# bpatchasaheb/mayaMatchMoveSolver

Hardware: AMD Instinct MI355X
Metric: LM iterations/sec + residuals/sec (markers x frames) at 1/2/4/8 MI355X; final RMS reproj error (higher is better)
Workload: dtype f64; 1 GPU; c4_500pose_50kbnd_200kobs; frames=500, cameras=1, bundles=50000, markers=50000, observations=200000, parameters=152991, residuals=400000, parallelism=single, solver=lmder fwd-FD delta=1e-4 tau=1 tol=1e-6

## Files before the change

include/mmba.h:

```cpp
#ifndef MMBA_H
#define MMBA_H

#include <stddef.h>
#include <stdint.h>

#ifdef __cplusplus
extern "C" {
#endif

#define MMBA_ABI_VERSION 12

#define MMBA_OK 0
#define MMBA_ERR_INVALID (-1)
#define MMBA_ERR_DEVICE (-2)
#define MMBA_ERR_UNSUPPORTED (-3)
#define MMBA_ERR_INTERRUPTED (-4)
#define MMBA_ERR_NO_DEVICE (-5)
#define MMBA_ERR_COMM (-6)

#define MMBA_SOLVER_CMINPACK_LMDIF 1
#define MMBA_SOLVER_CMINPACK_LMDER 2

#define MMBA_SCENE_GRAPH_MAYA_DAG 1
#define MMBA_SCENE_GRAPH_MM_SCENE_GRAPH 2
// ... 178 lines not shown
                                       double offset, double scale);
double mmba_param_internal_to_external(double value, double xmin, double xmax,
                                       double offset, double scale);

int mmba_context_create(int device, mmba_context **out);
int mmba_context_create_multi(const int *devices, int ndevices, mmba_context **out);
int mmba_context_num_devices(const mmba_context *ctx);
void mmba_context_destroy(mmba_context *ctx);
int mmba_context_synchronize(mmba_context *ctx);
int mmba_host_alloc(size_t bytes, void **out);
void mmba_host_free(void *p);

int mmba_plan_create(mmba_context *ctx, const mmba_problem *prob,
                     const mmba_options *opt, mmba_plan **out);
void mmba_plan_destroy(mmba_plan *plan);

typedef struct mmba_comm mmba_comm;
int mmba_comm_unique_id(unsigned char out_id[128]);
int mmba_comm_create_rccl(mmba_context *ctx, int rank, int nranks,
                          const unsigned char unique_id[128], mmba_comm **out);
int mmba_comm_create_local(int nranks, mmba_comm **out);
void mmba_comm_destroy(mmba_comm *comm);
int mmba_comm_count(const mmba_comm *comm);
int mmba_plan_create_sharded(mmba_context *ctx, const mmba_problem *prob,
                             const mmba_options *opt, mmba_comm *comm, mmba_plan **out);
int mmba_plan_num_shards(const mmba_plan *plan);
int mmba_shard_layout(int32_t num_frames, int32_t num_obs, const int32_t *obs_frame,
                      const int32_t *obs_bundle, int32_t num_bundles, int32_t nranks,
                      int32_t *bounds_out , int32_t *bundle_owner_out);

int mmba_plan_set_attr_values(mmba_plan *plan, const double *attr_values);

int mmba_plan_measure(mmba_plan *plan, const double *x, double *fvec_out,
                      double *err_user_out, double *err_dist_out,
                      double *avg_min_max_out );

int mmba_plan_reproject(mmba_plan *plan, const double *x, double *point_xy_out,
                        double *marker_xy_out);

int mmba_plan_jacobian(mmba_plan *plan, const double *x, double *fjac);

int mmba_plan_solve(mmba_plan *plan, double *x_inout, double *fvec_out,
                    double *err_user_out, double *err_dist_out,
                    mmba_result *res, const mmba_callbacks *cb,
                    mmba_trace *trace);

int mmba_plan_outputs(mmba_plan *plan, double *fvec_out, double *err_user_out,
                      double *err_dist_out);

int mmba_solve_per_frame(mmba_context *ctx, const mmba_problem *prob,
                         const mmba_options *opt, double *x_inout,
                         mmba_result *results , int32_t max_concurrency,
                         const mmba_callbacks *cb);

int mmba_plan_solve_per_frame(mmba_plan *plan, double *x_inout, mmba_result *results,
                              const mmba_callbacks *cb);

int mmba_solve(mmba_context *ctx, const mmba_problem *prob,
               const mmba_options *opt, double *x_inout, double *fvec_out,
               double *err_user_out, double *err_dist_out, mmba_result *res,
               const mmba_callbacks *cb, mmba_trace *trace);

typedef struct mmba_kernel_stats {
    double jac_ms_avg;
    double jac_bytes;
    int32_t jac_launches;
    double resid_ms_avg;
    double resid_bytes;
    int32_t resid_launches;
    double chol_ms_avg;
    double chol_flops;
    int32_t chol_launches;
    int32_t reduced_dim;
    int32_t reduced_kind;
    int32_t dataflow_fallback;
    int32_t shards_replicated;
    int32_t spec_replays;
    int32_t band_solver;
    int32_t band_levels;
    int32_t band_block;
    double chol_flops_alg;
    int32_t pre_handbacks;
    int32_t ne_split_launches;
} mmba_kernel_stats;
int mmba_plan_kernel_stats(mmba_plan *plan, int enable_timing,
                           mmba_kernel_stats *out);

#define MMBA_PATH_PCR 1
#define MMBA_PATH_SHARD_BCR 2
#define MMBA_PATH_BCR_DATAFLOW 3
#define MMBA_PATH_BCR_GRID 4
#define MMBA_PATH_DENSE 5
#define MMBA_PATH_PERFRAME_BATCH 6
#define MMBA_PATH_LOCAL_RING 7
#define MMBA_PATH_PROBE 8
#define MMBA_PATH_SHARD_SEP 9
#define MMBA_PATH_TRIAL_RECORDS 10
#define MMBA_PATH_LENS_CF 11
#define MMBA_PATH_DEST_LANE 12
#define MMBA_PATH_FAULT_SHARD 13
#define MMBA_PATH_COMM_TIMEOUT_MS 14
#define MMBA_PATH_STALL_SHARD 15
#define MMBA_PATH_PCR_CHAIN 16
#define MMBA_PATH_BACKSUB_ONEPASS 17
#define MMBA_PATH_JB_RECOMPUTE 18
#define MMBA_PATH_NE_CF_SPLIT 19
#define MMBA_PATH_RED_BD 20
#define MMBA_PATH_HANDBACK_DMA 21
#define MMBA_PATH_PRE_HANDBACK 22
#define MMBA_PATH_PRE_SCHUR 23
#define MMBA_PATH_BACKSUB_GROUP 24
#define MMBA_PATH_NUM 25
int mmba_debug_set_path(int key, int value);

int mmba_debug_band_solve(mmba_context *ctx, int nb, int w, int nG, int P, const double *S,
                          const double *r, double *x, double *ynorm2, int *parts_used);
int mmba_debug_comm_allreduce(mmba_context *ctx, mmba_comm *comm, double *buf, int count,
                              int op);
int mmba_debug_dgemm(mmba_context *ctx, int tri, int in_place, int M, int N, int K,
                     const double *A, int lda, const double *B, int ldb, double *C, int ldc,
                     double alpha, double beta);

int mmba_debug_reduced_residual(mmba_plan *plan, const double *x, double lam, double *relres);

int mmba_debug_damped_step(mmba_plan *plan, const double *x, double lam, double *step_out,
                           double *g_out, double *diag_out, double *fjac_out);

#ifdef __cplusplus
}
#endif

#endif
```

mayamatchmovesolver_amd/abi.py:

```python
import ctypes as C

MMBA_OK = 0
MMBA_ERR_INVALID = -1
MMBA_ERR_DEVICE = -2
MMBA_ERR_UNSUPPORTED = -3
MMBA_ERR_INTERRUPTED = -4
MMBA_ERR_NO_DEVICE = -5
MMBA_ERR_COMM = -6

SOLVER_TYPE_CMINPACK_LMDIF = 1
SOLVER_TYPE_CMINPACK_LMDER = 2
SCENE_GRAPH_MODE_MAYA_DAG = 1
SCENE_GRAPH_MODE_MM_SCENE_GRAPH = 2
AUTO_DIFF_TYPE_FORWARD = 0
AUTO_DIFF_TYPE_CENTRAL = 1
ROBUST_LOSS_TYPE_TRIVIAL = 0
ROBUST_LOSS_TYPE_SOFT_L_ONE = 1
ROBUST_LOSS_TYPE_CAUCHY = 2
ABI_VERSION = 12

PATH_PCR = 1
PATH_SHARD_BCR = 2
PATH_BCR_DATAFLOW = 3
PATH_BCR_GRID = 4
PATH_DENSE = 5
PATH_PERFRAME_BATCH = 6
PATH_LOCAL_RING = 7
PATH_PROBE = 8
PATH_SHARD_SEP = 9
PATH_TRIAL_RECORDS = 10
PATH_LENS_CF = 11
PATH_DEST_LANE = 12
PATH_FAULT_SHARD = 13
PATH_COMM_TIMEOUT_MS = 14
PATH_STALL_SHARD = 15
PATH_PCR_CHAIN = 16
PATH_BACKSUB_ONEPASS = 17
PATH_JB_RECOMPUTE = 18
PATH_NE_CF_SPLIT = 19
PATH_RED_BD = 20
PATH_HANDBACK_DMA = 21
PATH_PRE_HANDBACK = 22
PATH_PRE_SCHUR = 23
PATH_BACKSUB_GROUP = 24
PATH_NUM = 25

FILM_FIT_FILL = 0
FILM_FIT_HORIZONTAL = 1
FILM_FIT_VERTICAL = 2
FILM_FIT_OVERSCAN = 3

ROO_XYZ, ROO_YZX, ROO_ZXY, ROO_XZY, ROO_YXZ, ROO_ZYX = range(6)

LENS_NONE = 0
LENS_3DE_CLASSIC = 1
LENS_3DE_RADIAL_STD_DEG4 = 2
LENS_3DE_ANAMORPHIC_STD_DEG4 = 3
LENS_3DE_ANAMORPHIC_STD_DEG4_RESCALED = 4

CAM_FILM_BACK_W_INCH = 0
CAM_FILM_BACK_H_INCH = 1
CAM_FOCAL_MM = 2
CAM_FILM_OFFSET_X_INCH = 3
CAM_FILM_OFFSET_Y_INCH = 4
CAM_NEAR_CLIP = 5
CAM_FAR_CLIP = 6
CAM_SCALE = 7
CAM_NUM_ATTRS = 8
LENS_NUM_ATTRS = 14

_i32p = C.POINTER(C.c_int32)
_i64p = C.POINTER(C.c_int64)
_f64p = C.POINTER(C.c_double)


class MmbaProblem(C.Structure):
    _fields_ = [
        ("num_frames", C.c_int32),
        ("num_attrs", C.c_int32),
        ("attr_animated", _i32p),
        ("attr_offset", _i64p),
        ("attr_values", _f64p),
        ("num_transforms", C.c_int32),
        ("tfm_parent", _i32p),
        ("tfm_rotate_order", _i32p),
        ("tfm_attrs", _i32p),
        ("num_cameras", C.c_int32),
        ("cam_tfm", _i32p),
        ("cam_attrs", _i32p),
        ("cam_film_fit", _i32p),
        ("cam_render_size", _i32p),
        ("cam_lens", _i32p),
        ("num_lenses", C.c_int32),
        ("lens_type", _i32p),
        ("lens_attrs", _i32p),
        ("num_bundles", C.c_int32),
        ("bnd_tfm", _i32p),
        ("num_markers", C.c_int32),
        ("mkr_cam", _i32p),
        ("mkr_bnd", _i32p),
        ("num_obs", C.c_int32),
        ("obs_marker", _i32p),
        ("obs_frame", _i32p),
        ("obs_xy", _f64p),
        ("obs_weight", _f64p),
        ("num_params", C.c_int32),
        ("param_attr", _i32p),
        ("param_frame", _i32p),
        ("param_min", _f64p),
        ("param_max", _f64p),
        ("param_offset", _f64p),
        ("param_scale", _f64p),
        ("param_weight", _f64p),
        ("num_stiff", C.c_int32),
        ("stiff_attr", _i32p),
        ("stiff_frame", _i32p),
        ("stiff_weight", _f64p),
        ("stiff_variance", _f64p),
        ("stiff_value", _f64p),
        ("num_smooth", C.c_int32),
        ("smooth_attr", _i32p),
        ("smooth_frame", _i32p),
        ("smooth_weight", _f64p),
        ("smooth_variance", _f64p),
        ("smooth_value", _f64p),
        ("cam_rs_value", _f64p),
        ("lens_input", _i32p),
        ("lens_input_values", _f64p),
# ... 18 lines not shown
        ("scene_graph_mode", C.c_int32),
        ("image_width", C.c_double),
        ("accept_only_better", C.c_int32),
        ("log_level", C.c_int32),
        ("robust_loss", C.c_int32),
        ("robust_loss_type", C.c_int32),
        ("robust_loss_scale", C.c_double),
        ("initial_error_given", C.c_int32),
        ("pad_opt0", C.c_int32),
        ("initial_error_avg", C.c_double),
    ]


class MmbaResult(C.Structure):
    _fields_ = [
        ("success", C.c_int32),
        ("reason_number", C.c_int32),
        ("iterations", C.c_int32),
        ("function_evals", C.c_int32),
        ("jacobian_evals", C.c_int32),
        ("outer_iterations", C.c_int32),
        ("user_interrupted", C.c_int32),
        ("error_is_better", C.c_int32),
        ("error_final", C.c_double),
        ("error_avg", C.c_double),
        ("error_min", C.c_double),
        ("error_max", C.c_double),
        ("error_initial_avg", C.c_double),
        ("error_rms", C.c_double),
        ("num_trace", C.c_int32),
        ("pad0", C.c_int32),
        ("time_solve_s", C.c_double),
        ("time_func_s", C.c_double),
        ("time_jac_s", C.c_double),
        ("time_linear_s", C.c_double),
    ]

    def as_dict(self):
        return {name: getattr(self, name) for name, _ in self._fields_ if name != "pad0"}


INTERRUPT_FN = C.CFUNCTYPE(C.c_int, C.c_void_p)
PROGRESS_FN = C.CFUNCTYPE(None, C.c_void_p, C.c_int)


class MmbaCallbacks(C.Structure):
    _fields_ = [
        ("interrupt", INTERRUPT_FN),
        ("progress", PROGRESS_FN),
        ("user", C.c_void_p),
    ]


class MmbaTrace(C.Structure):
    _fields_ = [
        ("fnorm", _f64p),
        ("capacity", C.c_int32),
        ("count", C.c_int32),
    ]


class MmbaKernelStats(C.Structure):
    _fields_ = [
        ("jac_ms_avg", C.c_double),
        ("jac_bytes", C.c_double),
        ("jac_launches", C.c_int32),
        ("resid_ms_avg", C.c_double),
        ("resid_bytes", C.c_double),
        ("resid_launches", C.c_int32),
        ("chol_ms_avg", C.c_double),
        ("chol_flops", C.c_double),
        ("chol_launches", C.c_int32),
        ("reduced_dim", C.c_int32),
        ("reduced_kind", C.c_int32),
        ("dataflow_fallback", C.c_int32),
        ("shards_replicated", C.c_int32),
        ("spec_replays", C.c_int32),
        ("band_solver", C.c_int32),
        ("band_levels", C.c_int32),
        ("band_block", C.c_int32),
        ("chol_flops_alg", C.c_double),
        ("pre_handbacks", C.c_int32),
        ("ne_split_launches", C.c_int32),
    ]

    def as_dict(self):
        return {name: getattr(self, name) for name, _ in self._fields_}


EXPORTED_SYMBOLS = [
    "mmba_abi_version",
    "mmba_device_count",
    "mmba_last_error",
    "mmba_options_default",
    "mmba_param_external_to_internal",
    "mmba_param_internal_to_external",
    "mmba_context_create",
    "mmba_context_create_multi",
    "mmba_context_num_devices",
    "mmba_plan_num_shards",
    "mmba_debug_damped_step",
    "mmba_debug_reduced_residual",
    "mmba_context_destroy",
    "mmba_context_synchronize",
    "mmba_host_alloc",
    "mmba_host_free",
    "mmba_plan_create",
    "mmba_plan_destroy",
    "mmba_comm_unique_id",
    "mmba_shard_layout",
    "mmba_comm_create_rccl",
    "mmba_comm_create_local",
    "mmba_comm_destroy",
    "mmba_comm_count",
    "mmba_plan_create_sharded",
    "mmba_plan_measure",
    "mmba_plan_reproject",
    "mmba_solve_per_frame",
    "mmba_plan_solve_per_frame",
    "mmba_plan_set_attr_values",
    "mmba_plan_jacobian",
    "mmba_plan_solve",
    "mmba_plan_outputs",
    "mmba_solve",
    "mmba_plan_kernel_stats",
    "mmba_debug_set_path",
    "mmba_debug_band_solve",
    "mmba_debug_comm_allreduce",
    "mmba_debug_dgemm",
]
```

mayamatchmovesolver_amd/csrc/mmba_api.cpp:

```cpp
#include <atomic>
#include <cfloat>
#include <cmath>
#include <cstring>
#include <string>

#include "mmba_geom.h"
#include "mmba_kernels.h"
#include "mmba_plan.h"

namespace mmba {
static thread_local std::string g_last_error;
void set_error(const std::string &msg) { g_last_error = msg; }

static_assert(MMBA_PATH_NUM == 25, "one initialiser per path key");
static std::atomic<int> g_path[MMBA_PATH_NUM] = {-1, -1, -1, -1, -1, -1, -1, -1, -1, -1, -1, -1, -1,
                                                 -1, -1, -1, -1, -1, -1, -1, -1, -1, -1, -1, -1};
int path_choice(int key) {
    return (key > 0 && key < MMBA_PATH_NUM) ? g_path[key].load() : -1;
}
}

using namespace mmba;

#define MMBA_GUARD(...)                               \
    try {                                             \
        __VA_ARGS__                                   \
    } catch (const DeviceError &) {                   \
        return MMBA_ERR_DEVICE;                       \
    } catch (const CommError &) {                     \
        return MMBA_ERR_COMM;                         \
    } catch (const Unsupported &u) {                  \
        set_error("unsupported: " + u.what);          \
        return MMBA_ERR_UNSUPPORTED;                  \
    } catch (const Invalid &v) {                      \
        set_error("invalid: " + v.what);              \
        return MMBA_ERR_INVALID;                      \
    } catch (const std::exception &e) {               \
        set_error(std::string("exception: ") + e.what()); \
        return MMBA_ERR_INVALID;                      \
    }

extern "C" {

int mmba_abi_version(void) { return MMBA_ABI_VERSION; }

int mmba_debug_set_path(int key, int value) {
    if (key <= 0 || key >= MMBA_PATH_NUM) return MMBA_ERR_INVALID;
    g_path[key].store(value < 0 ? -1 : value);
    return MMBA_OK;
}

int mmba_shard_layout(int32_t num_frames, int32_t num_obs, const int32_t *obs_frame,
                      const int32_t *obs_bundle, int32_t num_bundles, int32_t nranks,
                      int32_t *bounds_out, int32_t *bundle_owner_out) {
    if (num_frames <= 0 || num_obs < 0 || nranks <= 0 || !bounds_out ||
        (num_obs > 0 && !obs_frame) || (bundle_owner_out && (!obs_bundle || num_bundles < 0)))
        return MMBA_ERR_INVALID;
    for (int i = 0; i < num_obs; ++i) {
        if (obs_frame[i] < 0 || obs_frame[i] >= num_frames) return MMBA_ERR_INVALID;
        if (bundle_owner_out && (obs_bundle[i] < 0 || obs_bundle[i] >= num_bundles))
            return MMBA_ERR_INVALID;
    }
    mmba::shard_layout(num_frames, num_obs, obs_frame, obs_bundle, num_bundles, nranks,
                       bounds_out, bundle_owner_out);
    return MMBA_OK;
}

const char *mmba_last_error(void) { return g_last_error.c_str(); }

int mmba_device_count(void) {
    int count = 0;
    if (hipGetDeviceCount(&count) != hipSuccess) return 0;
    int ok = 0;
    for (int d = 0; d < count; ++d) {
        hipDeviceProp_t prop;
        if (hipGetDeviceProperties(&prop, d) != hipSuccess) continue;
        if (std::strncmp(prop.gcnArchName, "gfx950", 6) == 0) ++ok;
    }
    return ok;
}

void mmba_options_default(mmba_options *o, int32_t solver_type) {
    if (!o) return;
    std::memset(o, 0, sizeof(*o));
    o->solver_type = solver_type ? solver_type : MMBA_SOLVER_CMINPACK_LMDER;
    o->iter_max = 100;
    o->tau = 1.0;
    o->eps1 = 1e-6;
    o->eps2 = 1e-6;
    o->eps3 = 1e-6;
    o->delta = 1e-4;
    o->auto_diff_type = MMBA_AUTO_DIFF_FORWARD;
    o->auto_param_scale = 1;
    o->scene_graph_mode = MMBA_SCENE_GRAPH_MAYA_DAG;
    o->image_width = 2048.0;
    o->accept_only_better = 1;
    o->log_level = 0;
}

// ... 223 lines not shown
                    mmba_trace *trace) {
    if (!plan || !x_inout) return MMBA_ERR_INVALID;
    if (plan->group)
        return group_plan_solve(plan, x_inout, fvec_out, err_user_out, err_dist_out, res, cb,
                                trace);
    MMBA_GUARD({
        MMBA_HIP(hipSetDevice(plan->impl.ctx->device));
        plan->impl.outputs_ready = false;
        const int rc =
            plan->impl.solve(x_inout, fvec_out, err_user_out, err_dist_out, res, cb, trace);
        plan->impl.outputs_ready = rc == MMBA_OK || rc == MMBA_ERR_INTERRUPTED;
        return rc;
    })
}

int mmba_plan_outputs(mmba_plan *plan, double *fvec_out, double *err_user_out,
                      double *err_dist_out) {
    if (plan && plan->group) return group_plan_outputs(plan, fvec_out, err_user_out, err_dist_out);
    if (!plan || !plan->impl.outputs_ready) return MMBA_ERR_INVALID;
    MMBA_GUARD({
        Plan &p = plan->impl;
        MMBA_HIP(hipSetDevice(p.ctx->device));
        if (fvec_out || err_user_out || err_dist_out)
            p.download_ref_order(p.d_f, p.d_eu, p.d_ed, fvec_out, err_user_out, err_dist_out);
        return MMBA_OK;
    })
}

int mmba_plan_set_attr_values(mmba_plan *plan, const double *attr_values) {
    if (!plan || !attr_values) return MMBA_ERR_INVALID;
    if (plan->group) return group_plan_set_attr_values(plan, attr_values);
    MMBA_GUARD({
        Plan &p = plan->impl;
        MMBA_HIP(hipSetDevice(p.ctx->device));
        std::memcpy(p.host_attr0.data(), attr_values, p.attr_bytes);
        MMBA_HIP(hipMemcpyAsync(p.d_attr0, p.host_attr0.data(), p.attr_bytes,
                                hipMemcpyHostToDevice, p.s));
        MMBA_HIP(hipStreamSynchronize(p.s));
        return MMBA_OK;
    })
}

int mmba_plan_solve_per_frame(mmba_plan *plan, double *x_inout, mmba_result *results,
                              const mmba_callbacks *cb) {
    if (!plan || !x_inout || !results) return MMBA_ERR_INVALID;
    if (plan->group) return group_plan_solve_per_frame(plan, x_inout, results, cb);
    MMBA_GUARD({
        MMBA_HIP(hipSetDevice(plan->impl.ctx->device));
        plan->impl.outputs_ready = false;
        return plan->impl.solve_frames(x_inout, results, cb);
    })
}

int mmba_solve(mmba_context *ctx, const mmba_problem *prob, const mmba_options *opt,
               double *x_inout, double *fvec_out, double *err_user_out, double *err_dist_out,
               mmba_result *res, const mmba_callbacks *cb, mmba_trace *trace) {
    mmba_plan *plan = nullptr;
    int rc = mmba_plan_create(ctx, prob, opt, &plan);
    if (rc != MMBA_OK) return rc;
    rc = mmba_plan_solve(plan, x_inout, fvec_out, err_user_out, err_dist_out, res, cb, trace);
    mmba_plan_destroy(plan);
    return rc;
}

int mmba_plan_kernel_stats(mmba_plan *plan, int enable_timing, mmba_kernel_stats *out) {
    if (!plan) return MMBA_ERR_INVALID;
    if (plan->group) return group_plan_kernel_stats(plan, enable_timing, out);
    Plan &p = plan->impl;
    if (out) {
        std::memset(out, 0, sizeof(*out));
        out->jac_launches = p.jac_n;
        out->jac_ms_avg = p.jac_n ? p.jac_ms / p.jac_n : 0.;
        out->resid_launches = p.resid_n;
        out->resid_ms_avg = p.resid_n ? p.resid_ms / p.resid_n : 0.;
        out->chol_launches = p.chol_n;
        out->chol_ms_avg = p.chol_n ? p.chol_ms / p.chol_n : 0.;
        out->reduced_dim = p.nR;
        out->reduced_kind = p.band ? (p.bs.use_bd ? 3 : 0) : (p.dense ? 2 : 1);
        out->dataflow_fallback = p.bs.df_off ? 1 : 0;
        out->shards_replicated = p.replicated ? 1 : 0;
        out->spec_replays = p.spec_replays;
        out->pre_handbacks = (int32_t)p.pre_handbacks;
        out->ne_split_launches = (int32_t)p.ne_split_launches;
        {
            const BandSolver &b = p.bs;
            out->band_solver = !p.band ? 0
                               : b.use_bd ? 5
                               : (b.pcr_int && !b.df_off) ? 4
                               : (b.use_pcr && !b.df_off) ? 3
                               : b.use_bcr ? 2
                               : 1;
        }
        double bj = 0.;
        {
            const double pc = p.ncf ? (double)p.nCF / p.ncf : 0.;
            const double pb = p.nB ? 3.0 * p.nB_solved / p.nB : 0.;
            const double pg = (double)std::min(p.nG, NGMAX);
            bj = 48.0 + 8.0 * pc * (pb + pg);
        }
        out->jac_bytes = bj * p.M;
        out->resid_bytes = 48.0 * p.M;
        if (p.band && p.bs.use_pcr && !p.bs.df_off) {
            const double K = p.bs.pcr.K;
            out->chol_flops = (double)p.bs.pcr.nblk *
                              (p.bs.pcr.nlev * (28.0 / 3.0 * K * K * K + 9.0 * K * K) + 2.0 * K * K);
        } else if (p.band && p.bs.use_bcr) {
            const double K = p.bs.bcr.K, G = p.bs.bcr.nG, N = p.bs.bcr.NR;
            out->chol_flops = (p.bs.bcr.nblk - 1) * (19.0 / 3.0 * K * K * K + 5.0 * G * K * K +
                                                     G * G * K + K * K) +
                              2.0 * N * N * N / 3.0;
        } else if (p.band && p.bs.use_bd) {
            const double pc = p.ncf ? (double)p.nCF / p.ncf : 0.;
            out->chol_flops = (double)p.nCF * pc * pc / 3.0;
        } else if (p.band) {
            out->chol_flops = (double)(p.nR - p.nG) * p.bw * p.bw;
        } else {
            out->chol_flops = (double)p.nRpad * p.nRpad * p.nRpad / 3.0;
        }
        {
            const double G = p.nG, nb = p.nR - p.nG;
            const double arrow = nb * G * (2.0 * p.bw + G) + G * G * G / 3.0 + 4.0 * G * G;
            if (p.band && p.bs.use_bd) {
                const double pc = p.ncf ? (double)p.nCF / p.ncf : 0.;
                out->chol_flops_alg = (double)p.ncf * (pc * pc * pc / 3.0 + 4.0 * pc * pc) +
                                      nb * G * (2.0 * pc + G) + G * G * G / 3.0 + 4.0 * G * G;
            } else if (p.band) {
                out->chol_flops_alg = nb * p.bw * p.bw + 4.0 * nb * p.bw + arrow;
            } else {
                const double N = p.nR;
                out->chol_flops_alg = N * N * N / 3.0 + 4.0 * N * N;
            }
            if (p.band && p.bs.use_pcr && !p.bs.df_off) {
                out->band_levels = p.bs.pcr.nlev;
                out->band_block = p.bs.pcr.K;
            } else if (p.band && p.bs.use_bcr) {
                out->band_levels = 0;
                for (int a = p.bs.bcr.nblk; a > 1; a = (a + 1) / 2) ++out->band_levels;
                out->band_block = p.bs.bcr.K;
            }
        }
    }
    p.timing = enable_timing != 0;
    if (enable_timing) {
        p.jac_ms = p.resid_ms = p.chol_ms = 0.;
        p.jac_n = p.resid_n = p.chol_n = 0;
        p.span_ctr[0] = p.span_ctr[1] = p.span_ctr[2] = 0;
    }
    return MMBA_OK;
}

int mmba_debug_reduced_residual(mmba_plan *plan, const double *x, double lam, double *relres) {
    if (!plan || !x || !relres || lam < 0.) return MMBA_ERR_INVALID;
    if (plan->group) {
        set_error("unsupported: reduced residual hook on a multi-device plan");
        return MMBA_ERR_UNSUPPORTED;
    }
    MMBA_GUARD({
        Plan &p = plan->impl;
        MMBA_HIP(hipSetDevice(p.ctx->device));
        p.outputs_ready = false;
        return p.reduced_residual(x, lam, relres);
    })
}

int mmba_debug_damped_step(mmba_plan *plan, const double *x, double lam, double *step_out,
                           double *g_out, double *diag_out, double *fjac_out) {
// ... 123 lines not shown
```

mayamatchmovesolver_amd/csrc/mmba_kernels.h:

```cpp
#pragma once

#include <vector>

#include "mmba_internal.h"

namespace mmba {

constexpr int NE_BND_TPB = 64;

void launch_param_prep(hipStream_t s, const DevProblem &P, const double *x, double *ext,
                       double *ext_pert, double *step, int solver_type, double delta,
                       double eps_dif);
void launch_set_attrs(hipStream_t s, const DevProblem &P, const double *ext);
void launch_param_set(hipStream_t s, const DevProblem &P, const double *x, double *ext,
                      double *ext_pert, double *step, int solver_type, double delta,
                      double eps_dif);
struct RedRow {
    int off, n, is_max, slot;
};
struct RedSpec {
    int nrows;
    int flag_slot;
    RedRow row[8];
};
// ... 23 lines not shown
int trial_blocks(const DevProblem &P);
void launch_reproject(hipStream_t s, const DevProblem &P, const double *recs, double *pts,
                      double *mkr);
void launch_residual(hipStream_t s, const DevProblem &P, const double *recs, double *f, double *eu,
                     double *ed, double *partial, double *out = nullptr,
                     unsigned int *ticket = nullptr, double *dist = nullptr);
void launch_dist_stats(hipStream_t s, const DevProblem &P, const double *ed, double *partial,
                       int nparts, int rstride, double *out);
struct RedTail {
    int on = 0;
    RedSpec spec{};
    const double *partial = nullptr;
    double *scalar = nullptr;
    int *flag = nullptr;
    double *host = nullptr;
    int host_n = 0;
    unsigned *ticket = nullptr;
};
void launch_residual_jp(hipStream_t s, const DevProblem &P, const double *recs, double *f,
                        double *eu, double *ed, double *partial, const double *J,
                        const int *jcol, const int *nloc, const double *pstep,
                        double *partial_jp, double *dist = nullptr, const RedTail &T = RedTail());
struct CentralB {
    const double *recs = nullptr, *brec = nullptr, *ext_pert = nullptr, *step = nullptr;
    const double *q15 = nullptr, *kap15 = nullptr;
};
void launch_param_central(hipStream_t s, const DevProblem &P, const double *x, double *ext_pertB,
                          double *stepB, double delta, double *count, double *c15 = nullptr);
void launch_b15_s(hipStream_t s, const double *fsq, double fn, double *out);
void launch_b15_combine(hipStream_t s, int n, const double *u, const double *c, const double *zu,
                        const double *zc, const double *sp, double *xs, double *kinv,
                        double *scalar, int fail_slot, const double *fail_prev);
void launch_b15_q(hipStream_t s, const DevProblem &P, const double *c, double *q15, double *kap15,
                  double *cr);
void launch_b15_rot(hipStream_t s, const DevProblem &P, const double *q15, const double *x,
                    double *out);
void launch_b15_accl(hipStream_t s, const DevProblem &P, const double *Acc, const double *q15,
                     const double *diag, double lam, double *AccL, double *diagL);
void launch_b15_unrot(hipStream_t s, const DevProblem &P, const double *Acc, const double *g,
                      const double *q15, double *adiag, double *u);
void launch_b15_unrot_J(hipStream_t s, const DevProblem &P, double *J, const double *q15);
void launch_b15_dnorm(hipStream_t s, int n, const double *x, const double *diag, double *out);
void launch_b15_newton(hipStream_t s, int n, const double *v, const double *zu, const double *zc,
                       const double *kinv, double *out);
void launch_b15_jp(hipStream_t s, int n, const double *xs, const double *u, const double *c,
                   const double *sp, double *out);
void launch_jacobian(hipStream_t s, const DevProblem &P, const double *recs,
                     const double *ext_pert, const double *step, int solver_type, double *J,
                     int *jcol, int *nloc, const int *stale_param, double *eu, double *ed,
                     int ncv = 0,
                     const double *f = nullptr,
                     const CentralB &CB = CentralB());
void launch_rows_eval(hipStream_t s, const DevProblem &P, double *fr, double *eur,
                      double *partial, int slot, const double *Jrow = nullptr,
                      const double *pstep = nullptr, double *partial_jp = nullptr);
void launch_rows_jac(hipStream_t s, const DevProblem &P, const double *ext,
                     const double *ext_pert, const double *step, const double *ext_pertB,
                     const double *stepB, int lmder, double *Jrow, double *eur, int last_param);
void launch_rows_ne(hipStream_t s, const DevProblem &P, const double *Jrow, const double *fr,
                    const int *p_own, double *Acc, double *Abb, double *aggbuf, double *g);
constexpr int NE_CF_SPLIT = 4;
constexpr int NE_CF_NT = 36;
struct NeEpi {
    int on = 0;
    int first = 0, mode = 1, do_xn = 0, do_gn = 0;
    double fnorm = 0.;
    const double *fnorm_sq = nullptr;
    const double *x = nullptr;
    double *diag = nullptr, *acnorm = nullptr, *partial = nullptr;
    int rstride = 0, cf_base = 0, bnd_base = 0;
    int fold = 0;
    RedSpec spec{};
    double *scalar = nullptr;
    unsigned *ticket = nullptr;
    const double *jb_recs = nullptr;
    int jb_lmder = 1;
    double *cf_part = nullptr;
    unsigned *cf_ticket = nullptr;
    double *Lb = nullptr, *tb = nullptr;
    int *fail = nullptr;
    const int *gate = nullptr;
    long long *probe = nullptr;
};
bool jac_ne_fusable(const DevProblem &P, int ncv);
void launch_jac_ne(hipStream_t s, const DevProblem &P, const double *recs, const double *step,
                   int solver_type, double *J, int *jcol, int *nloc, const int *stale_param,
                   double *eu, double *ed, double *Acc, double *g, const NeEpi &E);
bool ne_epilogue_fusable(const DevProblem &P);
bool launch_ne(hipStream_t s, const DevProblem &P, const double *J, const int *jcol,
               const int *nloc, const double *f, double *Acc, double *Acg, double *Abb,
               double *Abg, double *aggbuf, double *g, double *glob_partial, int glob_chunk,
               const NeEpi &epi = NeEpi(), bool cf_done = false);
void launch_colnorms(hipStream_t s, const DevProblem &P, const double *Acc, const double *Abb,
                     const double *aggbuf, double *acnorm, double *g);
void launch_bundle_factor(hipStream_t s, const DevProblem &P, const double *Abb,
                          const double *Abg, const double *g, const double *diag, double lam,
                          double *Lb, double *tb, double *Wg, int *fail);
void launch_schur_obs(hipStream_t s, const DevProblem &P, const double *J, const double *Lb,
                      double *W, const RedSpec *red = nullptr, const double *partial = nullptr,
                      double *scalar = nullptr, const int *gate = nullptr);
void launch_schur_obs_rs(hipStream_t s, const DevProblem &PV, int Mr, const int *nloc,
                         const int *vobs, const int *vcoff, const double *J, const double *Lb,
                         double *W);
void launch_schur_init(hipStream_t s, const DevProblem &P, const double *Acc, const double *Acg,
                       const double *Agg, const double *g, const double *diag, double lam,
                       const SView &V, int npad, double *rhs, const RedSpec *red = nullptr,
                       const double *partial = nullptr, double *scalar = nullptr);
void launch_schur_pairs(hipStream_t s, const DevProblem &P, const double *W, const double *Wg,
                        const double *tb, const SView &V, double *rhs);
void launch_chol_panel(hipStream_t s, double *S, const int *slot, int NT, int k, const int *rows,
                       int nrows, double *Linv, int *fail);
void launch_chol_update(hipStream_t s, double *S, const int *slot, int NT, int k,
                        const int2 *pairs, int npairs);
void launch_trsv_fwd(hipStream_t s, const double *S, const int *slot, int NT, int k,
                     const int *rows, int nrows, const double *Linv, double *r, double *y);
void launch_trsv_bwd(hipStream_t s, const double *S, const int *slot, int NT, int k,
                     const int *cols, int ncols, const double *Linv, double *y, double *x);
void launch_trsv_fwd_all(hipStream_t s, const double *S, const int *slot, int NT,
                         const int *rows_off, const int *rows, const double *Linv, double *r,
                         double *y);
void launch_trsv_bwd_all(hipStream_t s, const double *S, const int *slot, int NT,
                         const int *cols_off, const int *cols, const double *Linv, double *y,
                         double *x);
struct SchurInitFold {
    int on;
    const double *Acc, *g, *diag;
    double lam;
};
bool launch_schur_dest(hipStream_t s, const DevProblem &P, const double *W, const int2 *dest,
                       const int *dest_off, int ndest, const int2 *pairs, const SView &V,
                       int pc_uniform, int assign_off, const double *tb = nullptr,
                       double *rhs = nullptr, SchurInitFold fold = SchurInitFold{},
                       const int *wave_list = nullptr, int n_wave = 0,
                       const int *lane_list = nullptr, int n_lane = 0);
void launch_schur_rhs(hipStream_t s, const DevProblem &P, const double *W, const double *tb,
                      const int *row_cf, double *rhs);
void launch_schur_glob(hipStream_t s, const DevProblem &P, const double *W, const double *Wg,
                       const double *tb, const SView &V, double *rhs);
void launch_backsub_bundle(hipStream_t s, const DevProblem &P, const double *W, const double *Wg,
                           const double *tb, const double *Lb, const double *xR, double *U,
                           double *x);
struct TrialFold {
    const double *x = nullptr, *diag = nullptr;
    double *wa1 = nullptr, *wa2 = nullptr, *wa3 = nullptr;
    double *ext = nullptr, *ext_pert = nullptr, *step = nullptr;
    int solver_type = 0;
    double delta = 0., eps_dif = 0.;
    const int *other = nullptr;
    int nother = 0;
    double *partial = nullptr;
    int rstride = 0;
    const int *own = nullptr;
    int rec = 0;
    double *recs = nullptr, *brec = nullptr;
    int group = 0;
    const int2 *bobs_rp = nullptr;
    int brec_fwd = 0;
};
bool trial_records_ok(const DevProblem &P);
int trial_fold_parts(const DevProblem &P, int nother, bool rec = false);
int trial_prep_rec_parts(const DevProblem &P, int nother);
void launch_trial_prep_rec(hipStream_t s, const DevProblem &P, const double *xs, const TrialFold &T);
void launch_obs_wtx(hipStream_t s, const DevProblem &P, const double *W, const double *xR,
                    double *U);
void launch_backsub_trial(hipStream_t s, const DevProblem &P, const double *W, const double *Wg,
                          const double *tb, const double *Lb, const double *xR, const double *U,
                          double *x, const TrialFold &T);
void launch_scatter_xR(hipStream_t s, const DevProblem &P, const double *xR, double *x);
void launch_newton_bundle(hipStream_t s, const DevProblem &P, const double *W, const double *Wg,
                          const double *Lb, const double *v, double *wR, double *usq,
                          double *un, double *gp);
void launch_gather_R(hipStream_t s, const DevProblem &P, const double *v, double *vR, int nRpad);
void band_factor(hipStream_t s, const BandSolver &B, int *fail, long long *probe);
void band_factor_forward(hipStream_t s, const BandSolver &B, int *fail, long long *probe,
                         const double *r, double *y);
void band_forward(hipStream_t s, const BandSolver &B, const double *r, double *y);
void band_backward(hipStream_t s, const BandSolver &B, const double *y, double *x);
void bcr_factor(hipStream_t s, const BandSolver &B, int *fail, long long *probe,
                const double *r = nullptr, double *y = nullptr);
void bcr_forward(hipStream_t s, const BandSolver &B, const double *r, double *y);
void bcr_backward(hipStream_t s, const BandSolver &B, const double *y, double *x);
void pcr_solve(hipStream_t s, const PcrDev &P, const double *r, double *x, double *xs, int *fail);
void pcr_rhs_dot(hipStream_t s, const PcrDev &P, const double *w, const int *mask, int *fail);
void pcr_rhs_mc(hipStream_t s, const PcrDev &P, const double *R, int ldr, int nc, double *Z,
                int ldz, int *fail);
void pcr_note_context(int dev, int delta);
int pcr_max_resident(int K);
int pcr_resident_wide(int K);
int pcr_grid(int nblk);
void bd_direct(hipStream_t s, const DevProblem &P, const BdDev &D, const double *Acc,
               const double *g, const double *diag, double lam, double *xR, double *xs,
               int *fail, double *scalar, int dn_slot, int fail_slot,
               const RedSpec *red = nullptr, const double *partial = nullptr);
void bd_factor_solve(hipStream_t s, const BdDev &D, int *fail, const double *r, double *y,
                     double *x, double *xs);
void bd_forward(hipStream_t s, const BdDev &D, const double *w, double *y);
void launch_sumsq(hipStream_t s, const double *a, const double *d, int n, double *partial,
                  int nparts, double *out, const int *mask = nullptr,
                  unsigned int *ticket = nullptr);
void launch_sumsq_div(hipStream_t s, const double *a, const double *d, int n, double *partial,
                      int nparts, double *out, const int *mask = nullptr,
                      unsigned int *ticket = nullptr);
void launch_sumsq_mix(hipStream_t s, const double *y, const double *v, int n, double *partial,
                      int nparts, double *out, const int *mask);
void launch_reduce_sum(hipStream_t s, const double *partial, int n, double *out);
void launch_gnorm(hipStream_t s, const double *g, const double *acnorm, int n, double fnorm,
                  double *partial, int nparts, double *out, const int *mask = nullptr,
                  unsigned int *ticket = nullptr);
void launch_jp_sumsq(hipStream_t s, const DevProblem &P, const double *J, const int *jcol,
                     const int *nloc, const double *p, double *partial, int nparts,
                     double *out, unsigned int *ticket = nullptr);
void launch_zero_flag(hipStream_t s, const double *acnorm, int n, const int *mask,
                      double *partial, int nparts, double *out, unsigned int *ticket = nullptr);
void launch_flag_to_scalar(hipStream_t s, int *flag, double *out);
void launch_keep_rows(hipStream_t s, double *v, int lo, int hi, int nCF, int nR, int root);
void launch_keep_mask(hipStream_t s, const double *src, const int *mask, int n, double *dst);
void launch_lm_step(hipStream_t s, int n, const double *xs, const double *x, const double *diag,
                    double *wa1, double *wa2, double *wa3);
void launch_diag_init(hipStream_t s, int n, const double *acnorm, double *diag, int first,
                      int mode);
void launch_newton_v(hipStream_t s, int n, const double *diag, const double *x, double dxnorm,
                     double *v);
void launch_handback_host(hipStream_t s, int Mg, int nrows, const int *dev_of_ref,
                          const double *f2, const double *eu2, const double *ed, double *hf,
                          double *heu, double *hed, const double *dec = nullptr,
                          const double *f2_trial = nullptr);
void launch_unpermute(hipStream_t s, int M, const int *ref_of_dev, const int *obs_own,
                      const double *f2,
                      const double *eu2, const double *ed, double *f2o, double *eu2o,
                      double *edo);

void launch_fold_ranks(hipStream_t s, const double *t, int nranks, double *out, int do_xn,
                       int do_gn);

void launch_batch_lm(hipStream_t s, const DevProblem &P, const BatchArgs &B, int nf_max);

void launch_dgemm_nt(hipStream_t s, bool tri, int M, int N, int Kd, const double *A, int lda,
                     const double *B, int ldb, double *C, int ldc, double alpha, double beta);

void launch_jacobian_rs(hipStream_t s, const DevProblem &P, const double *ext_pert,
// ... 8 lines not shown
```

mayamatchmovesolver_amd/csrc/mmba_kernels.hip:

```cpp
#include <cfloat>
#include <cstdlib>

#include "mmba_geom.h"
#include "mmba_kernels.h"
#include "mmba_red_dev.h"

namespace mmba {

MMBA_DEV bool own_obs(const DevProblem &P, int i) { return !P.obs_own || P.obs_own[i]; }
MMBA_DEV bool own_cf(const DevProblem &P, int cf) { return !P.cf_own || P.cf_own[cf]; }
MMBA_DEV bool own_bnd(const DevProblem &P, int b) { return !P.bnd_own || P.bnd_own[b]; }
MMBA_DEV bool own_mask(const int *m, int i) { return !m || m[i]; }

__device__ __forceinline__ int xcd_remap(int b, int G) {
    const int x = b & 7, idx = b >> 3, q = G >> 3, r = G & 7;
    return x * q + min(x, r) + idx;
}

template <bool MAX>
__device__ __forceinline__ void finish_blocks(double v, double *partial, double *out,
                                              unsigned int *ticket, int blk = -1) {
    if (blk < 0) blk = blockIdx.x;
    __shared__ int last;
    __shared__ double red[256];
// ... 10 lines not shown
    if (!ticket) return;
    __syncthreads();
    if (!last) return;
    __threadfence();
    double a = 0.;
    for (int i = threadIdx.x; i < (int)gridDim.x; i += blockDim.x) {
        const double q = __hip_atomic_load(&partial[i], __ATOMIC_RELAXED, __HIP_MEMORY_SCOPE_AGENT);
        a = MAX ? fmax(a, q) : a + q;
    }
    red[threadIdx.x] = a;
    __syncthreads();
    for (int w = 128; w > 0; w >>= 1) {
        if (threadIdx.x < w)
            red[threadIdx.x] = MAX ? fmax(red[threadIdx.x], red[threadIdx.x + w])
                                   : red[threadIdx.x] + red[threadIdx.x + w];
        __syncthreads();
    }
    if (threadIdx.x == 0) {
        *out = red[0];
        __hip_atomic_store(ticket, 0u, __ATOMIC_RELAXED, __HIP_MEMORY_SCOPE_AGENT);
    }
}

__device__ __forceinline__ void bundle_chol3(double (&A)[3][3], double (&rhs)[3],
                                             const double (&dd)[3], int pb, double lam, int b,
                                             double *Lb, double *tb, int *fail,
                                             double (*Lo)[3] = nullptr, double *ilo = nullptr) {
#pragma unroll
    for (int a = 0; a < 3; ++a) {
        if (a < pb) {
            const double d = dd[a];
            A[a][a] += lam * (d * d);
            if (A[a][a] == 0.) {
                A[a][a] = 1.;
                rhs[a] = 0.;
            }
        }
    }
    double L[3][3] = {}, il[3];
    bool ok = true;
#pragma unroll
    for (int j = 0; j < 3; ++j) {
        double s = A[j][j];
#pragma unroll
        for (int k = 0; k < j; ++k) s -= L[j][k] * L[j][k];
        if (!(s > 0.)) {
            ok = false;
            s = 1.;
        }
        L[j][j] = sqrt(s);
        il[j] = 1.0 / L[j][j];
#pragma unroll
        for (int i = j + 1; i < 3; ++i) {
            double t = A[i][j];
#pragma unroll
            for (int k = 0; k < j; ++k) t -= L[i][k] * L[j][k];
            L[i][j] = t * il[j];
        }
    }
    if (!ok) atomicOr(fail, 1);
#pragma unroll
    for (int a = 0; a < 3; ++a)
#pragma unroll
        for (int c = 0; c < 3; ++c) Lb[(size_t)b * 9 + a * 3 + c] = (a < pb) ? L[a][c] : 0.;
    double t[3];
#pragma unroll
    for (int a = 0; a < 3; ++a) {
        double s = rhs[a];
#pragma unroll
        for (int k = 0; k < a; ++k) s -= L[a][k] * t[k];
        t[a] = s * il[a];
    }
    for (int a = 0; a < 3; ++a) tb[(size_t)b * 3 + a] = t[a];
    if (Lo) {
#pragma unroll
        for (int a = 0; a < 3; ++a) {
            ilo[a] = il[a];
#pragma unroll
            for (int c = 0; c < 3; ++c) Lo[a][c] = L[a][c];
        }
    }
}

__device__ __forceinline__ double reduce_row_w64(const double *partial, const RedRow &rw) {
    const bool mx = rw.is_max != 0;
    const int t = threadIdx.x & 63;
    double s[4];
    constexpr int JB = 6;
    if (rw.n <= 256 * JB) {
        double q[4][JB];
#pragma unroll
        for (int k = 0; k < 4; ++k)
#pragma unroll
            for (int j = 0; j < JB; ++j) {
                const int i = t + 64 * k + 256 * j;
                q[k][j] = i < rw.n ? partial[rw.off + i] : 0.;
            }
#pragma unroll
        for (int k = 0; k < 4; ++k) {
            double v = 0.;
#pragma unroll
            for (int j = 0; j < JB; ++j)
                if (t + 64 * k + 256 * j < rw.n) v = mx ? fmax(v, q[k][j]) : v + q[k][j];
            s[k] = v;
        }
    } else {
#pragma unroll
        for (int k = 0; k < 4; ++k) {
            double v = 0.;
            for (int i = t + 64 * k; i < rw.n; i += 256) {
                const double q = partial[rw.off + i];
                v = mx ? fmax(v, q) : v + q;
            }
            s[k] = v;
        }
    }
    const double a0 = mx ? fmax(s[0], s[2]) : s[0] + s[2];
    const double a1 = mx ? fmax(s[1], s[3]) : s[1] + s[3];
    double r = mx ? fmax(a0, a1) : a0 + a1;
#pragma unroll
    for (int w = 32; w > 0; w >>= 1) {
        const double o = __shfl_down(r, w);
        if (t < w) r = mx ? fmax(r, o) : r + o;
    }
    return r;
}

constexpr int RED_ROWS = 8;
__device__ __forceinline__ void reduce_rows_sc1(const RedSpec &spec, const double *partial,
                                                double *scalar) {
    __shared__ double red[RED_ROWS][256];
    const int nr = spec.nrows;
    double sv[RED_ROWS];
#pragma unroll
    for (int r = 0; r < RED_ROWS; ++r) {
        sv[r] = 0.;
        if (r < nr) {
            const RedRow rw = spec.row[r];
            const bool mx = rw.is_max != 0;
            for (int i = threadIdx.x; i < rw.n; i += blockDim.x) {
                const double q = ld_sc1(&partial[rw.off + i]);
                sv[r] = mx ? fmax(sv[r], q) : sv[r] + q;
            }
        }
    }
#pragma unroll
    for (int r = 0; r < RED_ROWS; ++r)
        if (r < nr) red[r][threadIdx.x] = sv[r];
    __syncthreads();
    for (int w = 128; w > 0; w >>= 1) {
        if (threadIdx.x < w) {
#pragma unroll
            for (int r = 0; r < RED_ROWS; ++r) {
                if (r >= nr) break;
                const bool mx = spec.row[r].is_max != 0;
                red[r][threadIdx.x] = mx ? fmax(red[r][threadIdx.x], red[r][threadIdx.x + w])
                                         : red[r][threadIdx.x] + red[r][threadIdx.x + w];
            }
        }
        __syncthreads();
    }
    if (threadIdx.x < nr) scalar[spec.row[threadIdx.x].slot] = red[threadIdx.x][0];
    __syncthreads();
}

__device__ __forceinline__ void tail_reduce(const RedSpec &spec, const double *partial,
                                            double *scalar, unsigned *ticket) {
    __shared__ unsigned last;
    asm volatile("s_waitcnt vmcnt(0)" ::: "memory");
    __syncthreads();
    if (threadIdx.x == 0)
        last = __hip_atomic_fetch_add(ticket, 1u, __ATOMIC_RELAXED, __HIP_MEMORY_SCOPE_AGENT) ==
               gridDim.x - 1;
    __syncthreads();
    if (!last) return;
    reduce_rows_sc1(spec, partial, scalar);
    if (threadIdx.x == 0) __hip_atomic_store(ticket, 0u, __ATOMIC_RELAXED, __HIP_MEMORY_SCOPE_AGENT);
}

__device__ __forceinline__ void tail_reduce_full(const RedTail &T) {
    __shared__ unsigned last;
    asm volatile("s_waitcnt vmcnt(0)" ::: "memory");
    __syncthreads();
    if (threadIdx.x == 0)
        last = __hip_atomic_fetch_add(T.ticket, 1u, __ATOMIC_RELAXED, __HIP_MEMORY_SCOPE_AGENT) ==
               gridDim.x - 1;
    __syncthreads();
    if (!last) return;
    reduce_rows_sc1(T.spec, T.partial, T.scalar);
    if (threadIdx.x == 0 && T.flag && T.spec.flag_slot >= 0) {
        T.scalar[T.spec.flag_slot] = (double)*T.flag;
        *T.flag = 0;
    }
    if (T.host) {
        asm volatile("s_waitcnt vmcnt(0)" ::: "memory");
        __syncthreads();
        for (int i = threadIdx.x; i < T.host_n; i += blockDim.x) T.host[i] = ld_sc1(&T.scalar[i]);
    }
    if (threadIdx.x == 0)
        __hip_atomic_store(T.ticket, 0u, __ATOMIC_RELAXED, __HIP_MEMORY_SCOPE_AGENT);
}

__device__ __forceinline__ void param_prep_one(const DevProblem &P, int p, double v, double *ext,
                                               double *ext_pert, double *step, int solver_type,
                                               double delta, double eps_dif) {
    const double xmin = P.p_min[p], xmax = P.p_max[p], off = P.p_off[p], sc = P.p_scale[p];
    ext[p] = int_to_ext(v, xmin, xmax, off, sc);
    double st;
// ... 700 lines not shown
        __syncthreads();
        for (int t = threadIdx.x; t < 2 * lm * NE_CHUNK; t += blockDim.x) {
            const int row = t / NE_CHUNK, o = t % NE_CHUNK;
            sJ[row][o] = (o < cnt) ? J[(size_t)row * M + c0 + o] : 0.;
        }
        if (nG > 0) {
            for (int t = threadIdx.x; t < NGMAX * NE_CHUNK; t += blockDim.x)
                sG[t / NE_CHUNK][t % NE_CHUNK] = -1;
            __syncthreads();
            for (int t = threadIdx.x; t < lm * NE_CHUNK; t += blockDim.x) {
                const int l = t / NE_CHUNK, o = t % NE_CHUNK;
                if (o >= cnt || l < pc || l >= nloc[c0 + o]) continue;
                const int p = jcol[(size_t)l * M + c0 + o];
                if (P.p_class[p] == PC_G) sG[P.p_pos[p] - nCF][o] = l;
            }
        }
        for (int t = threadIdx.x; t < NE_CHUNK; t += blockDim.x) {
            sF[0][t] = (t < cnt) ? f[2 * (c0 + t)] : 0.;
            sF[1][t] = (t < cnt) ? f[2 * (c0 + t) + 1] : 0.;
        }
        __syncthreads();
        if (kind == 0) {
            for (int o = 0; o < cnt; ++o)
                acc += sJ[2 * ea][o] * sJ[2 * eb][o] + sJ[2 * ea + 1][o] * sJ[2 * eb + 1][o];
        } else if (kind == 1) {
            for (int o = 0; o < cnt; ++o)
                acc += sJ[2 * ea][o] * sF[0][o] + sJ[2 * ea + 1][o] * sF[1][o];
        } else if (kind == 2) {
            for (int o = 0; o < cnt; ++o) {
                const int l = sG[eb][o];
                if (l >= 0)
                    acc += sJ[2 * ea][o] * sJ[2 * l][o] + sJ[2 * ea + 1][o] * sJ[2 * l + 1][o];
            }
        }
    }
    double *A = &Acc[(size_t)cf * PCMAX * PCMAX];
    if (kind == 0) {
        A[ea * PCMAX + eb] = acc;
        A[eb * PCMAX + ea] = acc;
    } else if (kind == 1) {
        g[P.cf_var_param[P.cf_var_off[cf] + 1 + ea]] = acc;
    } else if (kind == 2) {
        Acg[((size_t)cf * PCMAX + ea) * NGMAX + eb] = acc;
    }
}

__device__ __forceinline__ double epi_param(const NeEpi &E, int p, double d, double gp, double &zf,
                                          double &xn, double &gm) {
    const double an = sqrt(d);
    E.acnorm[p] = an;
    double dg = E.diag[p];
    if (E.mode != 2) {
        if (E.first) dg = an == 0. ? 1. : an;
        dg = fmax(dg, an);
        E.diag[p] = dg;
    }
    if (an == 0.) zf = 1.;
    if (E.do_xn) {
        const double v = dg * E.x[p];
        xn += v * v;
    }
    if (E.do_gn && an != 0.) {
        const double fn = E.fnorm_sq ? sqrt(*E.fnorm_sq) : E.fnorm;
        if (fn != 0.) gm = fmax(gm, fabs((gp / fn) / an));
    }
    return dg;
}

__device__ __forceinline__ void epi_store(const NeEpi &E, int col, double zf, double xn,
                                          double gm) {
    E.partial[col] = zf;
    E.partial[E.rstride + col] = xn;
    E.partial[2 * E.rstride + col] = gm;
}

struct EpiPre {
    int p;
    double dg;
    double xv;
    double fn;
};
template <int PC>
__device__ __forceinline__ EpiPre epi_preload(const DevProblem &P, const NeEpi &E, int cf,
                                              int lane) {
    EpiPre q{-1, 0., 0., 0.};
    if (!E.on || lane >= PC) return q;
    q.p = P.cf_var_param[P.cf_var_off[cf] + 1 + lane];
    q.dg = E.diag[q.p];
    if (E.do_xn) q.xv = E.x[q.p];
    if (E.do_gn) q.fn = E.fnorm_sq ? sqrt(*E.fnorm_sq) : E.fnorm;
    return q;
}
__device__ __forceinline__ void epi_param_pre(const NeEpi &E, const EpiPre &q, double d, double gp,
                                              double &zf, double &xn, double &gm) {
    const double an = sqrt(d);
    E.acnorm[q.p] = an;
    double dg = q.dg;
    if (E.mode != 2) {
        if (E.first) dg = an == 0. ? 1. : an;
        dg = fmax(dg, an);
        E.diag[q.p] = dg;
    }
    if (an == 0.) zf = 1.;
    if (E.do_xn) {
        const double v = dg * q.xv;
        xn += v * v;
    }
    if (E.do_gn && an != 0.) {
        if (q.fn != 0.) gm = fmax(gm, fabs((gp / q.fn) / an));
    }
}
template <int PC>
__device__ __forceinline__ void epi_params_wave(const DevProblem &P, const NeEpi &E, int cf,
                                                int lane, double d, double gp, const EpiPre &q) {
    double zf = 0., xn = 0., gm = 0.;
    if (lane < PC) epi_param_pre(E, q, d, gp, zf, xn, gm);
    double Z = 0., X = 0., G = 0.;
#pragma unroll
    for (int a = 0; a < PC; ++a) {
        const double za = __shfl(zf, a), xa = __shfl(xn, a), ga = __shfl(gm, a);
        if (za != 0.) Z = 1.;
        X += xa;
        G = fmax(G, ga);
    }
    if (lane == 0) epi_store(E, E.cf_base + cf, Z, X, G);
}


template <int PC, int NW, int NG>
__device__ __forceinline__ void ne_cf_u_body(const DevProblem &P, const double *__restrict__ J,
                                             const int *__restrict__ jcol,
                                             const int *__restrict__ nloc,
                                             const double *__restrict__ f, double *Acc,
                                             double *Acg, double *g, const NeEpi &E, int blk,
                                             int nblk_cf) {
    constexpr int NCC = PC * (PC + 1) / 2, NE = NCC + PC, NT = NE + PC * NG;
    __shared__ double wsum[NW][NT];
    const int cf = xcd_remap(blk, nblk_cf);
    if (!own_cf(P, cf) || P.cf_pc[cf] != PC) {
        if (E.on && threadIdx.x == 0) epi_store(E, E.cf_base + cf, 0., 0., 0.);
        return;
    }
    const int o0 = P.cf_obs_off[cf], o1 = P.cf_obs_off[cf + 1];
    const size_t M = P.M;
    const int nCF = P.nR - P.nG;
    const int tid = threadIdx.x, lane = tid & 63, wv = tid >> 6;
    const EpiPre epq = epi_preload<PC>(P, E, cf, lane);
    double acc[NT];
#pragma unroll
    for (int e = 0; e < NT; ++e) acc[e] = 0.;
    for (int i = o0 + tid; i < o1; i += 64 * NW) {
        double jx[PC], jy[PC];
#pragma unroll
        for (int a = 0; a < PC; ++a) {
            jx[a] = J[(2 * a) * M + i];
            jy[a] = J[(2 * a + 1) * M + i];
        }
        const double fx = f[2 * i], fy = f[2 * i + 1];
        int e = 0;
#pragma unroll
        for (int a = 0; a < PC; ++a)
#pragma unroll
            for (int c = a; c < PC; ++c) acc[e++] += jx[a] * jx[c] + jy[a] * jy[c];
#pragma unroll
        for (int a = 0; a < PC; ++a) acc[NCC + a] += jx[a] * fx + jy[a] * fy;
        if constexpr (NG > 0) {
            double gx[NG], gy[NG];
#pragma unroll
            for (int q = 0; q < NG; ++q) gx[q] = gy[q] = 0.;
            const int nl = nloc[i];
            for (int l = PC; l < nl; ++l) {
                const int p = jcol[(size_t)l * M + i];
                if (P.p_class[p] != PC_G) continue;
// ... 84 lines not shown
        double jx[PC], jy[PC];
#pragma unroll
        for (int a = 0; a < PC; ++a) {
            jx[a] = J[(2 * a) * M + i];
            jy[a] = J[(2 * a + 1) * M + i];
        }
        const double fx = f[2 * i], fy = f[2 * i + 1];
        int e = 0;
#pragma unroll
        for (int a = 0; a < PC; ++a)
#pragma unroll
            for (int c = a; c < PC; ++c) acc[e++] += jx[a] * jx[c] + jy[a] * jy[c];
#pragma unroll
        for (int a = 0; a < PC; ++a) acc[NCC + a] += jx[a] * fx + jy[a] * fy;
    }
#pragma unroll
    for (int e = 0; e < NT; ++e) {
        double v = acc[e];
#pragma unroll
        for (int off = 32; off > 0; off >>= 1) v += __shfl_xor(v, off);
        if (lane == 0) wsum[wv][e] = v;
    }
    __syncthreads();
    double *mine = E.cf_part + ((size_t)cf * NS + part) * NE_CF_NT;
    for (int e = tid; e < NT; e += 64 * NW) {
        double v = wsum[0][e];
#pragma unroll
        for (int w = 1; w < NW; ++w) v += wsum[w][e];
        st_sc1(&mine[e], v);
    }
    asm volatile("s_waitcnt vmcnt(0)" ::: "memory");
    __syncthreads();
    if (tid == 0)
        last_s = (__hip_atomic_fetch_add(&E.cf_ticket[cf], 1u, __ATOMIC_ACQ_REL,
                                         __HIP_MEMORY_SCOPE_AGENT) %
                  NS) == NS - 1;
    __syncthreads();
    if (!last_s) return;
    __builtin_amdgcn_fence(__ATOMIC_ACQUIRE, "agent");
    const double *all = E.cf_part + (size_t)cf * NS * NE_CF_NT;
    for (int e = tid; e < NT; e += 64 * NW) {
        double t[NS];
#pragma unroll
        for (int q = 0; q < NS; ++q) t[q] = ld_sc1(&all[(size_t)q * NE_CF_NT + e]);
        double v = t[0];
#pragma unroll
        for (int q = 1; q < NS; ++q) v += t[q];
        fin[e] = v;
    }
    __syncthreads();
    double *A = &Acc[(size_t)cf * PCMAX * PCMAX];
    for (int e = tid; e < NT; e += 64 * NW) {
        const double v = fin[e];
        if (e < NCC) {
            int a = 0, rem = e;
            while (rem >= PC - a) {
                rem -= PC - a;
                ++a;
            }
            const int c = a + rem;
            A[a * PCMAX + c] = v;
            A[c * PCMAX + a] = v;
        } else {
            g[P.cf_var_param[P.cf_var_off[cf] + 1 + (e - NCC)]] = v;
        }
    }
    if (E.on && wv == 0) {
        const int ed = lane * PC - lane * (lane - 1) / 2;
        epi_params_wave<PC>(P, E, cf, lane, lane < PC ? fin[ed] : 0., lane < PC ? fin[NCC + lane] : 0.,
                            epq);
    }
}

template <int PC, int NW, int NG>
__global__ void __launch_bounds__(64 * NW) k_ne_cf_u(DevProblem P, const double *__restrict__ J,
                                                     const int *__restrict__ jcol,
                                                     const int *__restrict__ nloc,
                                                     const double *__restrict__ f, double *Acc,
                                                     double *Acg, double *g, NeEpi E) {
    ne_cf_u_body<PC, NW, NG>(P, J, jcol, nloc, f, Acc, Acg, g, E, blockIdx.x, gridDim.x);
}


template <int PC, int NW, bool GEN>
__global__ void __launch_bounds__(64 * NW) k_jac_ne_u(
    DevProblem P, const double *__restrict__ recs, const double *__restrict__ step,
    int solver_type, double *__restrict__ J, int *__restrict__ jcol, int *__restrict__ nloc,
    const int *__restrict__ stale_param, double *__restrict__ eu, double *__restrict__ ed,
    double *Acc, double *g, NeEpi E) {
    constexpr int NCC = PC * (PC + 1) / 2, NE = NCC + PC;
    __shared__ double wsum[NW][NE];
    __shared__ double sRec[(PC + 1) * CAMREC];
    __shared__ int sPv[PC];
    __shared__ double sSt[PC];
    __shared__ int sHdr[3];
    if (E.gate && __hip_atomic_load(E.gate, __ATOMIC_RELAXED, __HIP_MEMORY_SCOPE_AGENT) == 0)
        return;
    const int cf = xcd_remap(blockIdx.x, gridDim.x);
    long long *pr = (E.probe && threadIdx.x == 0) ? E.probe + 5 * (size_t)cf : nullptr;
    if (pr) pr[0] = (long long)wall_clock64();
    const int o0 = P.cf_obs_off[cf], o1 = P.cf_obs_off[cf + 1];
    const int tid = threadIdx.x, lane = tid & 63, wv = tid >> 6;
    const bool lmder = solver_type == MMBA_SOLVER_CMINPACK_LMDER;
    const bool solved = P.cf_pc[cf] == PC && own_cf(P, cf);
    {
        const int voff = P.cf_var_off[cf];
        const int nv = min(P.cf_var_off[cf + 1] - voff - 1, PC);
        for (int t = tid; t < (nv + 1) * CAMREC; t += 64 * NW)
            sRec[t] = recs[(size_t)voff * CAMREC + t];
        if (tid < PC) {
            const int p = tid < nv ? P.cf_var_param[voff + 1 + tid] : -1;
            sPv[tid] = p;
            sSt[tid] = tid < nv ? step[p] : 1.;
        }
        if (tid == 0) {
            const int fr = P.cf_frame[cf];
            sHdr[0] = nv;
            sHdr[1] = fr;
            sHdr[2] = stale_param[fr];
        }
    }
    __syncthreads();
    if (pr) pr[1] = (long long)wall_clock64();
    JacCf<PC> C;
    C.rcf = sRec;
#pragma unroll
    for (int v = 0; v < PC; ++v) {
        C.pv[v] = sPv[v];
        C.st[v] = sSt[v];
    }
    C.nv = sHdr[0];
    C.fr = sHdr[1];
    C.pstale = sHdr[2];
    double acc[NE];
#pragma unroll
    for (int e = 0; e < NE; ++e) acc[e] = 0.;
    for (int i = o0 + tid; i < o1; i += 64 * NW) {
        double jx[PC], jy[PC], fx, fy;
        int z = 0;
        asm volatile("" : "+s"(z));
        C.rcf = sRec + z;
        jac_obs_u<PC, GEN>(P, i, C, lmder, J, jcol, nloc, eu, ed, jx, jy, fx, fy);
        int e = 0;
#pragma unroll
        for (int a = 0; a < PC; ++a)
#pragma unroll
            for (int c = a; c < PC; ++c) acc[e++] += jx[a] * jx[c] + jy[a] * jy[c];
#pragma unroll
        for (int a = 0; a < PC; ++a) acc[NCC + a] += jx[a] * fx + jy[a] * fy;
    }
    if (pr) pr[2] = (long long)wall_clock64();
    if (!solved) {
        if (E.on && tid == 0) epi_store(E, E.cf_base + cf, 0., 0., 0.);
        if (pr) pr[3] = pr[2];
        return;
    }
#pragma unroll
    for (int e = 0; e < NE; ++e) {
        double v = acc[e];
#pragma unroll
        for (int off = 32; off > 0; off >>= 1) v += __shfl_xor(v, off);
        if (lane == 0) wsum[wv][e] = v;
    }
    __syncthreads();
    double *A = &Acc[(size_t)cf * PCMAX * PCMAX];
    for (int e = tid; e < NE; e += 64 * NW) {
        double v = wsum[0][e];
#pragma unroll
        for (int w = 1; w < NW; ++w) v += wsum[w][e];
        if (e < NCC) {
            int a = 0, rem = e;
            while (rem >= PC - a) {
                rem -= PC - a;
                ++a;
            }
            const int c = a + rem;
            A[a * PCMAX + c] = v;
            A[c * PCMAX + a] = v;
        } else {
            g[P.cf_var_param[P.cf_var_off[cf] + 1 + (e - NCC)]] = v;
        }
    }
    if (E.on && (tid >> 6) == 0) {
        const int ln = tid & 63;
        double d = 0., gp = 0.;
        if (ln < PC) {
            const int ed2 = ln * PC - ln * (ln - 1) / 2;
            d = wsum[0][ed2];
            gp = wsum[0][NCC + ln];
#pragma unroll
            for (int w = 1; w < NW; ++w) {
                d += wsum[w][ed2];
                gp += wsum[w][NCC + ln];
            }
        }
        epi_params_wave<PC>(P, E, cf, ln, d, gp, epi_preload<PC>(P, E, cf, ln));
    }
    if (pr) {
        pr[3] = (long long)wall_clock64();
        unsigned xcc;
        asm volatile("s_getreg_b32 %0, hwreg(HW_REG_XCC_ID)" : "=s"(xcc));
        pr[4] = (long long)(xcc & 0xf);
    }
}

__global__ void __launch_bounds__(NE_BND_TPB) k_ne_bnd_jb(DevProblem P, double *Abb, double *g,
                                                          NeEpi E) {
    __shared__ double red[3][NE_BND_TPB];
    if (E.gate && __hip_atomic_load(E.gate, __ATOMIC_RELAXED, __HIP_MEMORY_SCOPE_AGENT) == 0)
        return;
    const int b = xcd_remap(blockIdx.x, gridDim.x) * blockDim.x + threadIdx.x;
    const int4 p4 = b < P.nB ? P.bnd_p4[b] : make_int4(-1, -1, -1, 0);
    const int pb = p4.w;
    double zf = 0., xn = 0., gm = 0.;
    if (pb > 0) {
        double A[PBMAX][PBMAX] = {};
        double gb[PBMAX] = {};
        const int q0 = P.bobs_off[b], q1 = P.bobs_off[b + 1];
        const double *__restrict__ br = &P.brec[(size_t)b * BREC];
        for (int qb = q0; qb < q1; qb += 4) {
            double4 u[4], v[4];
            if (E.jb_recs) {
                const double bp0[3] = {br[0], br[1], br[2]};
#pragma unroll
                for (int r = 0; r < 4; ++r) {
                    if (qb + r >= q1) break;
                    const int i = P.bobs[qb + r];
                    const double *__restrict__ rec0 = &E.jb_recs[(size_t)P.cf_var_off[P.obs_cf[i]] * CAMREC];
                    const double mx = P.obs_xy[2 * i], my = P.obs_xy[2 * i + 1], sw = P.obs_sqrtw[i];
                    const double2 f0 = residual_e(rec0, bp0, mx, my, sw, P.mode, P.image_width);
                    double jb[6] = {0., 0., 0., 0., 0., 0.};
#pragma unroll
                    for (int a = 0; a < 3; ++a) {
                        if (a < pb) {
                            const double bq[3] = {br[3 + 3 * a], br[4 + 3 * a], br[5 + 3 * a]};
                            const double2 rr = residual_e(rec0, bq, mx, my, sw, P.mode, P.image_width);
                            const double st = br[12 + a];
                            jb[2 * a] = E.jb_lmder ? (rr.x - f0.x) * st : (rr.x - f0.x) / st;
                            jb[2 * a + 1] = E.jb_lmder ? (rr.y - f0.y) * st : (rr.y - f0.y) / st;
                        }
                    }
                    u[r] = make_double4(jb[0], jb[1], jb[2], jb[3]);
                    v[r] = make_double4(jb[4], jb[5], f0.x, f0.y);
                }
            } else {
#pragma unroll
                for (int r = 0; r < 4; ++r) {
                    if (qb + r < q1) {
                        const double4 *src = reinterpret_cast<const double4 *>(&P.JB[(size_t)(qb + r) * 8]);
                        u[r] = src[0];
                        v[r] = src[1];
                    }
                }
            }
#pragma unroll
            for (int r = 0; r < 4; ++r) {
                if (qb + r >= q1) break;
                const double jx[3] = {u[r].x, u[r].z, v[r].x}, jy[3] = {u[r].y, u[r].w, v[r].y};
                const double fx = v[r].z, fy = v[r].w;
#pragma unroll
                for (int a = 0; a < 3; ++a) {
#pragma unroll
                    for (int c = 0; c < 3; ++c) A[a][c] += jx[a] * jx[c] + jy[a] * jy[c];
                    gb[a] += jx[a] * fx + jy[a] * fy;
                }
            }
        }
        double *Ab = &Abb[(size_t)b * 9];
#pragma unroll
        for (int a = 0; a < PBMAX; ++a)
#pragma unroll
            for (int c = 0; c < PBMAX; ++c) Ab[a * 3 + c] = (a < pb && c < pb) ? A[a][c] : 0.;
        g[p4.x] = gb[0];
        if (pb > 1) g[p4.y] = gb[1];
        if (pb > 2) g[p4.z] = gb[2];
        double dd[3] = {0., 0., 0.};
        if (E.on) {
            double zo = 0., xo = 0., go = 0.;
            dd[0] = epi_param(E, p4.x, A[0][0], gb[0], zo, xo, go);
// ... 321 lines not shown
    for (int p = blockIdx.x * blockDim.x + threadIdx.x; p < P.n; p += gridDim.x * blockDim.x) {
        const int cls = P.p_class[p];
        double d = 0.;
        double gp;
        if (cls == PC_CF) {
            const int cf = P.p_blk[p];
            const int a = P.p_pos[p] - P.cf_roff[cf];
            d = Acc[(size_t)cf * PCMAX * PCMAX + a * PCMAX + a];
            gp = g[p];
        } else if (cls == PC_B) {
            const int b = P.p_blk[p];
            const int a = P.p_pos[p];
            d = Abb[(size_t)b * 9 + a * 3 + a];
            gp = g[p];
        } else {
            const int gi = P.p_pos[p] - (P.nR - P.nG);
            d = Agg[gi * NGMAX + gi];
            gp = gG[gi];
            g[p] = gp;
        }
        if (c15) {
            if (cls == PC_CF) {
                d = adiag15[p];
                gp = u15[p];
            }
            const double cp = c15[p];
            d = fmax(d + 2. * cp * gp + s15v * cp * cp, 0.);
            gp = gp + s15v * cp;
            gfull[p] = gp;
        }
        const double an = sqrt(d);
        acnorm[p] = an;
        double dg = diag[p];
        if (mode != 2) {
            if (first) dg = an == 0. ? 1. : an;
            dg = fmax(dg, an);
            diag[p] = dg;
        }
        if (own_mask(mask, p)) {
            if (an == 0.) zf = 1.;
            if (do_xn) {
                const double v = dg * x[p];
                xn += v * v;
            }
            if (do_gn && an != 0.) gm = fmax(gm, fabs((gp / fnorm) / an));
        }
    }
    block_partial<true>(zf, red, partial);
    __syncthreads();
    block_partial<false>(xn, red, partial + rstride);
    __syncthreads();
    block_partial<true>(gm, red, partial + 2 * rstride);
}

__global__ void __launch_bounds__(256) k_trial_prep(
    DevProblem P, const double *__restrict__ xs, const double *__restrict__ x,
    const double *__restrict__ diag, double *wa1, double *wa2, double *wa3, double *ext,
    double *ext_pert, double *step, int solver_type, double delta, double eps_dif,
    const int *__restrict__ mask, double *partial, int rstride) {
    __shared__ double red[256];
    double pn = 0., xn = 0.;
    for (int j = blockIdx.x * blockDim.x + threadIdx.x; j < P.n; j += gridDim.x * blockDim.x) {
        const double st = -xs[j];
        const double dj = diag[j];
        const double xj = x[j] + st;
        const double w3 = dj * st;
        wa1[j] = st;
        wa2[j] = xj;
        wa3[j] = w3;
        param_prep_one(P, j, xj, ext, ext_pert, step, solver_type, delta, eps_dif);
        set_attr_one(P, j, ext[j]);
        if (own_mask(mask, j)) {
            pn += w3 * w3;
            const double v = dj * xj;
            xn += v * v;
        }
    }
    block_partial<false>(pn, red, partial);
    __syncthreads();
    block_partial<false>(xn, red, partial + rstride);
}

__device__ void lm_decide(const LmDec &d, double *scalar) {
    const double p1 = .1, p5 = .5, p25 = .25, p75 = .75, p0001 = 1e-4;
    const double epsmch = DBL_EPSILON;
    double fnorm = d.f0 ? sqrt(scalar[d.s_f0]) : d.fnorm;
    double delta = d.delta, xnorm = d.xnorm, par = d.par, gnorm = d.gnorm;
    int info = 0, go = 0;
    double ratio = 0.;
    bool taken = true;
    if (d.spec) {
        if (d.first) {
            xnorm = sqrt(scalar[d.s_xn2]);
            delta = d.factor * xnorm;
            if (delta == 0.) delta = d.factor;
        }
        gnorm = fnorm != 0. ? scalar[d.s_gnorm] : 0.;
        if (gnorm <= d.gtol) {
            info = 4;
            taken = false;
        } else {
            const double fl = scalar[d.s_fail];
            const bool ok0 = fl == 0.;
            const double dxnorm = ok0 ? sqrt(scalar[d.s_dnorm]) : HUGE_VAL;
            const double fp = dxnorm - delta;
            taken = fl < 2. && fp <= p1 * delta;
            par = 0.;
        }
    }
    if (taken) {
        const double pnorm = sqrt(scalar[d.s_pnorm]);
        if (d.first) delta = fmin(delta, pnorm);
        const double fnorm1 = sqrt(scalar[d.s_fnorm]);
        double actred = -1.;
        if (p1 * fnorm1 < fnorm) {
            const double d1 = fnorm1 / fnorm;
            actred = 1. - d1 * d1;
        }
        const double temp1 = sqrt(scalar[d.s_jp]) / fnorm;
        const double temp2 = (sqrt(par) * pnorm) / fnorm;
        const double prered = temp1 * temp1 + temp2 * temp2 / p5;
        const double dirder = -(temp1 * temp1 + temp2 * temp2);
        if (prered != 0.) ratio = actred / prered;
        if (ratio <= p25) {
            double temp;
            if (actred >= 0.)
                temp = p5;
            else
                temp = p5 * dirder / (dirder + p5 * actred);
            if (p1 * fnorm1 >= fnorm || temp < p1) temp = p1;
            delta = temp * fmin(delta, pnorm / p1);
            par /= temp;
        } else if (par == 0. || ratio >= p75) {
            delta = pnorm / p5;
            par = p5 * par;
        }
        const bool accept = ratio >= p0001;
        if (accept) xnorm = sqrt(scalar[d.s_xn2t]);
        if (fabs(actred) <= d.ftol && prered <= d.ftol && p5 * ratio <= 1.) info = 1;
        if (delta <= d.xtol * xnorm) info = 2;
        if (fabs(actred) <= d.ftol && prered <= d.ftol && p5 * ratio <= 1. && info == 2) info = 3;
        if (info == 0) {
            if (d.nfev >= d.maxfev) info = 5;
            if (fabs(actred) <= epsmch && prered <= epsmch && p5 * ratio <= 1.) info = 6;
            if (delta <= epsmch * xnorm) info = 7;
            if (gnorm <= epsmch) info = 8;
        }
        go = (accept && info == 0) ? 1 : 0;
    }
    scalar[d.s_out] = go;
    scalar[d.s_out + 1] = ratio;
    scalar[d.s_out + 2] = delta;
    scalar[d.s_out + 3] = par;
    scalar[d.s_out + 4] = taken ? info : -100 - info;
    __hip_atomic_store(d.gate, go, __ATOMIC_RELAXED, __HIP_MEMORY_SCOPE_AGENT);
}

__global__ void __launch_bounds__(256) k_reduce_multi(const double *__restrict__ partial,
                                                      RedSpec spec, double *scalar, int *flag,
                                                      double *host, int host_n,
                                                      unsigned *ticket, unsigned *host_seq,
                                                      unsigned seq, const LmDec dec) {
    __shared__ double red[256];
    const RedRow rw = spec.row[blockIdx.x];
    const double v = reduce_row_block<false>(partial, rw, red);
    if (threadIdx.x == 0) {
        scalar[rw.slot] = v;
        if (blockIdx.x == 0 && flag && spec.flag_slot >= 0) {
            scalar[spec.flag_slot] = (double)*flag;
            *flag = 0;
        }
    }
    if (!host && !dec.on) return;
    __shared__ unsigned last;
    if (threadIdx.x == 0) {
        const unsigned t = __hip_atomic_fetch_add(ticket, 1u, __ATOMIC_ACQ_REL,
                                                  __HIP_MEMORY_SCOPE_AGENT);
        last = t == gridDim.x - 1;
    }
    __syncthreads();
    if (!last) return;
    __builtin_amdgcn_fence(__ATOMIC_ACQUIRE, "agent");
    if (dec.on) {
        if (threadIdx.x == 0) lm_decide(dec, scalar);
        __syncthreads();
        __builtin_amdgcn_fence(__ATOMIC_SEQ_CST, "workgroup");
    }
    if (!host) {
        if (threadIdx.x == 0)
            __hip_atomic_store(ticket, 0u, __ATOMIC_RELAXED, __HIP_MEMORY_SCOPE_AGENT);
        return;
    }
    if (threadIdx.x < 64) {
        for (int i = threadIdx.x; i < host_n; i += 64)
            host[i] = __hip_atomic_load(&scalar[i], __ATOMIC_RELAXED, __HIP_MEMORY_SCOPE_AGENT);
        if (host_seq) {
            __threadfence_system();
            if (threadIdx.x == 0)
                __hip_atomic_store(host_seq, seq, __ATOMIC_RELEASE, __HIP_MEMORY_SCOPE_SYSTEM);
        }
    }
    if (threadIdx.x == 0) __hip_atomic_store(ticket, 0u, __ATOMIC_RELAXED, __HIP_MEMORY_SCOPE_AGENT);
}

__global__ void k_bundle_factor(DevProblem P, const double *__restrict__ Abb,
                                const double *__restrict__ Abg, const double *__restrict__ g,
                                const double *__restrict__ diag, double lam, double *Lb,
                                double *tb, double *Wg, int *fail) {
    const int b = xcd_remap(blockIdx.x, gridDim.x) * blockDim.x + threadIdx.x;
    if (b >= P.nB) return;
    const int pb = P.bnd_pb[b];
    if (pb == 0) return;
    const int po = P.bnd_par_off[b];
    double A[3][3], rhs[3], dd[3];
#pragma unroll
    for (int a = 0; a < 3; ++a) {
#pragma unroll
        for (int c = 0; c < 3; ++c)
            A[a][c] = (a < pb && c < pb) ? Abb[(size_t)b * 9 + a * 3 + c] : (a == c ? 1. : 0.);
        rhs[a] = 0.;
        dd[a] = 0.;
        if (a < pb) {
            const int p = P.bnd_par[po + a];
            dd[a] = diag[p];
            rhs[a] = g[p];
        }
    }
    double L[3][3], il[3];
    bundle_chol3(A, rhs, dd, pb, lam, b, Lb, tb, fail, L, il);
    for (int q = 0; q < P.nG; ++q) {
        double w[3];
#pragma unroll
        for (int a = 0; a < 3; ++a) {
            double s = a < pb ? Abg[((size_t)b * PBMAX + a) * NGMAX + q] : 0.;
#pragma unroll
            for (int k = 0; k < a; ++k) s -= L[a][k] * w[k];
            w[a] = s * il[a];
        }
// ... 614 lines not shown
    double s[3] = {tb[(size_t)b * 3], tb[(size_t)b * 3 + 1], tb[(size_t)b * 3 + 2]};
    for (int q = P.bobs_off[b]; q < P.bobs_off[b + 1]; ++q) {
        double u[3];
        if (W) {
            const int i = P.bobs[q];
            const int cf = P.obs_cf[i];
            const int pc = min(P.cf_pc[cf], P.wst / 3);
            const int r0 = P.cf_roff[cf];
            const double *row = &W[widx(P, 0, i)];
            u[0] = u[1] = u[2] = 0.;
            for (int a = 0; a < pc; ++a) {
                const double xv = xR[r0 + a];
                for (int c = 0; c < 3; ++c) u[c] += row[a * 3 + c] * xv;
            }
        } else {
            const double4 uu = reinterpret_cast<const double4 *>(U)[P.bobs[q]];
            u[0] = uu.x;
            u[1] = uu.y;
            u[2] = uu.z;
        }
        s[0] -= u[0];
        s[1] -= u[1];
        s[2] -= u[2];
    }
    for (int q = 0; q < nG; ++q) {
        const double xv = xR[nCF + q];
        for (int c = 0; c < 3; ++c) s[c] -= Wg[((size_t)b * NGMAX + q) * 3 + c] * xv;
    }
    double L[3][3];
    for (int a = 0; a < 3; ++a)
        for (int c = 0; c < 3; ++c) L[a][c] = Lb[(size_t)b * 9 + a * 3 + c];
    double xb[3] = {0., 0., 0.};
#pragma unroll
    for (int a = 2; a >= 0; --a) {
        if (a >= pb) continue;
        double t = s[a];
#pragma unroll
        for (int k = a + 1; k < 3; ++k)
            if (k < pb) t -= L[k][a] * xb[k];
        xb[a] = t / L[a][a];
    }
    const int po = P.bnd_par_off[b];
#pragma unroll
    for (int a = 0; a < 3; ++a)
        if (a < pb) x[P.bnd_par[po + a]] = xb[a];
}

__device__ __forceinline__ void trial_one_pre(const DevProblem &P, const TrialFold &T, int j,
                                              double xsj, double dj, double x0, double &pn,
                                              double &xn) {
    const double st = -xsj;
    const double xj = x0 + st;
    const double w3 = dj * st;
    T.wa1[j] = st;
    T.wa2[j] = xj;
    T.wa3[j] = w3;
    param_prep_one(P, j, xj, T.ext, T.ext_pert, T.step, T.solver_type, T.delta, T.eps_dif);
    set_attr_one(P, j, T.ext[j]);
    if (own_mask(T.own, j)) {
        pn += w3 * w3;
        const double v = dj * xj;
        xn += v * v;
    }
}

__device__ __forceinline__ void trial_one(const DevProblem &P, const TrialFold &T, int j,
                                          double xsj, double &pn, double &xn) {
    const double st = -xsj;
    const double dj = T.diag[j];
    const double xj = T.x[j] + st;
    const double w3 = dj * st;
    T.wa1[j] = st;
    T.wa2[j] = xj;
    T.wa3[j] = w3;
    param_prep_one(P, j, xj, T.ext, T.ext_pert, T.step, T.solver_type, T.delta, T.eps_dif);
    set_attr_one(P, j, T.ext[j]);
    if (own_mask(T.own, j)) {
        pn += w3 * w3;
        const double v = dj * xj;
        xn += v * v;
    }
}

__global__ void __launch_bounds__(64) k_backsub_trial(DevProblem P, const double *__restrict__ U,
                                                      const double *__restrict__ W,
                                                      const double *__restrict__ Wg,
                                                      const double *__restrict__ tb,
                                                      const double *__restrict__ Lb,
                                                      const double *__restrict__ xR, double *x,
                                                      int nbb, TrialFold T) {
    __shared__ double red[256];
    double pn = 0., xn = 0.;
    if ((int)blockIdx.x < nbb) {
        const int b = xcd_remap(blockIdx.x, nbb) * blockDim.x + threadIdx.x;
        const int pb = b < P.nB ? P.bnd_pb[b] : 0;
        if (pb > 0) {
            const int nG = P.nG;
            const int nCF = P.nR - nG;
            double s[3] = {tb[(size_t)b * 3], tb[(size_t)b * 3 + 1], tb[(size_t)b * 3 + 2]};
            const int q0 = P.bobs_off[b], q1 = P.bobs_off[b + 1];
            const int po = P.bnd_par_off[b];
            int jj[3] = {-1, -1, -1};
            double dgj[3] = {0., 0., 0.}, x0j[3] = {0., 0., 0.};
#pragma unroll
            for (int a = 0; a < 3; ++a)
                if (a < pb) jj[a] = P.bnd_par[po + a];
#pragma unroll
            for (int a = 0; a < 3; ++a)
                if (a < pb) {
                    dgj[a] = T.diag[jj[a]];
                    x0j[a] = T.x[jj[a]];
                }
            if (W) {
                for (int q = q0; q < q1; ++q) {
                    double u[3];
                    const int i = P.bobs[q];
                    const int cf = P.obs_cf[i];
                    const int pc = min(P.cf_pc[cf], P.wst / 3);
                    const int r0 = P.cf_roff[cf];
                    const double *row = &W[widx(P, 0, i)];
                    u[0] = u[1] = u[2] = 0.;
                    for (int a = 0; a < pc; ++a) {
                        const double xv = xR[r0 + a];
                        for (int c = 0; c < 3; ++c) u[c] += row[a * 3 + c] * xv;
                    }
                    s[0] -= u[0];
                    s[1] -= u[1];
                    s[2] -= u[2];
                }
            } else {
                const double4 *U4 = reinterpret_cast<const double4 *>(U);
                for (int qb = q0; qb < q1; qb += 4) {
                    double4 uu[4];
#pragma unroll
                    for (int k = 0; k < 4; ++k)
                        if (qb + k < q1) uu[k] = U4[P.bobs[qb + k]];
#pragma unroll
                    for (int k = 0; k < 4; ++k)
                        if (qb + k < q1) {
                            s[0] -= uu[k].x;
                            s[1] -= uu[k].y;
                            s[2] -= uu[k].z;
                        }
                }
            }
            for (int q = 0; q < nG; ++q) {
                const double xv = xR[nCF + q];
                for (int c = 0; c < 3; ++c) s[c] -= Wg[((size_t)b * NGMAX + q) * 3 + c] * xv;
            }
            double L[3][3];
            for (int a = 0; a < 3; ++a)
                for (int c = 0; c < 3; ++c) L[a][c] = Lb[(size_t)b * 9 + a * 3 + c];
            double xb[3] = {0., 0., 0.};
#pragma unroll
            for (int a = 2; a >= 0; --a) {
                if (a >= pb) continue;
                double t = s[a];
#pragma unroll
                for (int k = a + 1; k < 3; ++k)
                    if (k < pb) t -= L[k][a] * xb[k];
                xb[a] = t / L[a][a];
            }
#pragma unroll
            for (int a = 0; a < 3; ++a)
                if (a < pb) {
                    const int j = jj[a];
                    x[j] = xb[a];
                    trial_one_pre(P, T, j, xb[a], dgj[a], x0j[a], pn, xn);
                }
        }
        if (T.rec && b < P.nB) bnd_record_thread(P, b, T.ext_pert, T.step, T.brec, 0);
    } else if (T.rec) {
        const int cf = ((int)blockIdx.x - nbb) * 4 + (int)(threadIdx.x >> 4);
        const int v = threadIdx.x & 15;
        int off = 0, nv = -1;
        if (cf < P.ncf) {
            off = P.cf_var_off[cf];
            nv = P.cf_var_off[cf + 1] - off - 1;
        }
        if (v < nv) {
            const int j = P.cf_var_param[off + 1 + v];
            trial_one(P, T, j, x[j], pn, xn);
        }
        __syncthreads();
        if (v <= nv) {
            const int p = P.cf_var_param[off + v];
            const long long ov_idx = p >= 0 ? P.p_vidx[p] : -1;
            const double ov_val = p >= 0 ? T.ext_pert[p] : 0.;
            camera_record_fast(P, cf, ov_idx, ov_val, &T.recs[(size_t)(off + v) * CAMREC],
                               p >= 0 ? P.p_attr[p] : -1);
        }
    } else {
        const int k = (blockIdx.x - nbb) * blockDim.x + threadIdx.x;
        if (k < T.nother) {
            const int j = T.other[k];
            trial_one(P, T, j, x[j], pn, xn);
        }
    }
    red[threadIdx.x] = pn;
    red[64 + threadIdx.x] = xn;
    __syncthreads();
    for (int w = 32; w > 0; w >>= 1) {
        if ((int)threadIdx.x < w) {
            red[threadIdx.x] += red[threadIdx.x + w];
            red[64 + threadIdx.x] += red[64 + threadIdx.x + w];
        }
        __syncthreads();
    }
    if (threadIdx.x == 0) {
        T.partial[blockIdx.x] = red[0];
        T.partial[T.rstride + blockIdx.x] = red[64];
    }
}

template <bool ONEPASS, bool W18>
__global__ void __launch_bounds__(256) k_backsub_trial_g(DevProblem P, const double *__restrict__ U,
                                                         const double *__restrict__ W,
                                                         const double *__restrict__ Wg,
                                                         const double *__restrict__ tb,
                                                         const double *__restrict__ Lb,
                                                         const double *__restrict__ xR, double *x,
                                                         int nbb, int nob, TrialFold T) {
    __shared__ double red[128];
    const int tid = threadIdx.x;
    const int pad = (nob + 7) & ~7;
    if ((int)blockIdx.x >= nob && (int)blockIdx.x < pad) return;
    const int bb = (int)blockIdx.x - pad, ob = (int)blockIdx.x;
    const int lb = bb >= 0 ? bb : nbb + ob;
    double pn = 0., xn = 0.;
    int leaf = tid < 64 ? tid : -1;
    if (bb >= 0) {
        const int k = tid & 3;
        const int b = xcd_remap(bb, nbb) * 64 + (tid >> 2);
        const bool live = b < P.nB;
        const bool fwd = T.rec && T.brec_fwd && P.bnd_vx;
        leaf = k == 0 ? (tid >> 2) : -1;
        int pb = 0, q0 = 0, q1 = 0, pcm = 0;
        int4 p4 = make_int4(-1, -1, -1, -1), vx = make_int4(-1, -1, -1, 0);
        double s[3] = {0., 0., 0.};
        double L[3][3] = {};
        if (live) {
            pb = P.bnd_pb[b];
            p4 = P.bnd_p4[b];
            q0 = P.bobs_off[b];
            q1 = P.bobs_off[b + 1];
#pragma unroll
            for (int a = 0; a < 3; ++a) s[a] = tb[(size_t)b * 3 + a];
#pragma unroll
            for (int a = 0; a < 3; ++a)
#pragma unroll
                for (int c = 0; c < 3; ++c) L[a][c] = Lb[(size_t)b * 9 + a * 3 + c];
            if (fwd) {
                vx = P.bnd_vx[b];
                pcm = P.bnd_pcomp[b];
            }
        }
        if (pb == 0) q1 = q0;
        const int j = k < pb ? (k == 0 ? p4.x : (k == 1 ? p4.y : p4.z)) : -1;
        double dg = 0., x0 = 0., xmin = 0., xmax = 0., off = 0., sc = 1.;
        long long vi = 0;
        bool own = false;
        if (j >= 0) {
            dg = T.diag[j];
            x0 = T.x[j];
            xmin = P.p_min[j];
            xmax = P.p_max[j];
            off = P.p_off[j];
            sc = P.p_scale[j];
            vi = P.p_vidx[j];
            own = own_mask(T.own, j);
        }
        int i = -1;
        int2 rp = make_int2(0, 0);
        if (q0 + k < q1) {
            i = P.bobs[q0 + k];
            if (ONEPASS) rp = T.bobs_rp[q0 + k];
        }
        const int pw = fwd ? p4.w : -1;
        double base[3] = {0., 0., 0.};
        if (pw >= 0) {
            int dm = 0;
#pragma unroll
            for (int a = 0; a < 3; ++a)
                if (a < pw) dm |= 1 << ((pcm >> (2 * a)) & 3);
            if (vx.x >= 0 && !(dm & 1)) base[0] = P.attr_val[vx.x];
            if (vx.y >= 0 && !(dm & 2)) base[1] = P.attr_val[vx.y];
            if (vx.z >= 0 && !(dm & 4)) base[2] = P.attr_val[vx.z];
        }
        const double4 *U4 = reinterpret_cast<const double4 *>(U);
        for (int qb = q0; qb < q1; qb += 4) {
            double u[3] = {0., 0., 0.};
            if (i >= 0) {
                if (ONEPASS && W18) {
                    const double2 *row = reinterpret_cast<const double2 *>(&W[(size_t)i * 18]);
                    double2 r2[9];
#pragma unroll
                    for (int t = 0; t < 9; ++t) r2[t] = row[t];
                    const int pc = min(rp.y, 6);
                    double xv[6];
#pragma unroll
                    for (int a = 0; a < 6; ++a) xv[a] = a < pc ? xR[rp.x + a] : 0.;
                    double w[18];
#pragma unroll
                    for (int t = 0; t < 9; ++t) {
                        w[2 * t] = r2[t].x;
                        w[2 * t + 1] = r2[t].y;
                    }
// ... 704 lines not shown
        partial[blockIdx.x] = red[0][0];
        partial[rstride + blockIdx.x] = red[1][0];
        partial[2 * rstride + blockIdx.x] = red[2][0];
    }
}

__global__ void __launch_bounds__(256) k_dist_stats_fin(const double *__restrict__ partial,
                                                        int n, int rstride, double *out) {
    __shared__ double red[3][256];
    double sm = 0., nmn = -DBL_MAX, mx = -0.0;
    for (int i = threadIdx.x; i < n; i += blockDim.x) {
        sm += partial[i];
        nmn = fmax(nmn, partial[rstride + i]);
        mx = fmax(mx, partial[2 * rstride + i]);
    }
    red[0][threadIdx.x] = sm;
    red[1][threadIdx.x] = nmn;
    red[2][threadIdx.x] = mx;
    __syncthreads();
    for (int w = 128; w > 0; w >>= 1) {
        if ((int)threadIdx.x < w) {
            red[0][threadIdx.x] += red[0][threadIdx.x + w];
            red[1][threadIdx.x] = fmax(red[1][threadIdx.x], red[1][threadIdx.x + w]);
            red[2][threadIdx.x] = fmax(red[2][threadIdx.x], red[2][threadIdx.x + w]);
        }
        __syncthreads();
    }
    if (threadIdx.x == 0) {
        out[0] = red[0][0];
        out[1] = red[1][0];
        out[2] = red[2][0];
    }
}

void launch_dist_stats(hipStream_t s, const DevProblem &P, const double *ed, double *partial,
                       int nparts, int rstride, double *out) {
    k_dist_stats<<<nparts, 256, 0, s>>>(P, ed, partial, rstride);
    k_dist_stats_fin<<<1, 256, 0, s>>>(partial, nparts, rstride, out);
}
void launch_jacobian(hipStream_t s, const DevProblem &P, const double *recs,
                     const double *ext_pert, const double *step, int solver_type, double *J,
                     int *jcol, int *nloc, const int *stale_param, double *eu, double *ed,
                     int ncv, const double *f, const CentralB &CB) {
    (void)f;
    if (P.rs) {
        launch_jacobian_rs(s, P, ext_pert, step, solver_type, J, jcol, nloc, stale_param, eu, ed);
        return;
    }
    constexpr bool uni = true;
#define MMBA_JAC_U(NCV, GEN)                                                                \
    do {                                                                                    \
        if (uni)                                                                            \
            k_jacobian_u<NCV, GEN, true><<<nblk(P.M, 128), 128, 0, s>>>(                    \
                P, recs, step, solver_type, J, jcol, nloc, stale_param, eu, ed);            \
        else                                                                                \
            k_jacobian_u<NCV, GEN, false><<<nblk(P.M, 128), 128, 0, s>>>(                   \
                P, recs, step, solver_type, J, jcol, nloc, stale_param, eu, ed);            \
    } while (0)
    if (ncv == 6 || ncv == 7) {
        if (ncv == 6) {
            if (P.all_bnd_fast) MMBA_JAC_U(6, false); else MMBA_JAC_U(6, true);
        } else {
            if (P.all_bnd_fast) MMBA_JAC_U(7, false); else MMBA_JAC_U(7, true);
        }
        return;
    }
#undef MMBA_JAC_U
    if (CB.recs)
        k_jacobian<true><<<nblk(P.M, 128), 128, 0, s>>>(P, recs, ext_pert, step, solver_type, J,
                                                      jcol, nloc, stale_param, eu, ed, CB);
    else if (P.lens_uniform == MMBA_LENS_3DE_CLASSIC)
        k_jacobian<false, MMBA_LENS_3DE_CLASSIC><<<nblk(P.M, 128), 128, 0, s>>>(
            P, recs, ext_pert, step, solver_type, J, jcol, nloc, stale_param, eu, ed, CB);
    else
        k_jacobian<false><<<nblk(P.M, 128), 128, 0, s>>>(P, recs, ext_pert, step, solver_type, J,
                                                       jcol, nloc, stale_param, eu, ed, CB);
}
bool jac_ne_fusable(const DevProblem &P, int ncv) {
    return P.nG == 0 && P.pc_uniform == ncv && (ncv == 6 || ncv == 7) &&
           P.nrows == 0 && !P.loss_on && P.ncf >= 256 && !P.rs;
}
void launch_jac_ne(hipStream_t s, const DevProblem &P, const double *recs, const double *step,
                   int solver_type, double *J, int *jcol, int *nloc, const int *stale_param,
                   double *eu, double *ed, double *Acc, double *g, const NeEpi &E) {
    if (P.ncf == 0) return;
    const long long per = (P.M + P.ncf - 1) / P.ncf;
    int nw = per > 1024 ? 8 : (per > 256 ? 4 : 2);
#define MMBA_JN(PC, NW, GEN)                                                                  \
    k_jac_ne_u<PC, NW, GEN><<<P.ncf, 64 * NW, 0, s>>>(P, recs, step, solver_type, J, jcol, nloc, \
                                                        stale_param, eu, ed, Acc, g, E)
#define MMBA_JN_NW(PC, GEN)                                         \
    do {                                                            \
        if (nw == 8) MMBA_JN(PC, 8, GEN);                           \
        else if (nw == 4) MMBA_JN(PC, 4, GEN);                      \
        else MMBA_JN(PC, 2, GEN);                                   \
    } while (0)
#define MMBA_JN_PC(PC)                                              \
    do {                                                            \
        if (P.all_bnd_fast) MMBA_JN_NW(PC, false);                  \
        else MMBA_JN_NW(PC, true);                                  \
    } while (0)
    if (P.pc_uniform == 6)
        MMBA_JN_PC(6);
    else
        MMBA_JN_PC(7);
#undef MMBA_JN_PC
#undef MMBA_JN_NW
#undef MMBA_JN
}
__global__ void k_fold_ranks(const double *__restrict__ t, int nranks, double *out, int do_xn,
                             int do_gn) {
    if (threadIdx.x != 0) return;
    out[0] = t[0];
    if (do_xn) out[1] = t[1];
    if (do_gn) {
        double g = 0.;
        for (int r = 0; r < nranks; ++r) g = fmax(g, t[2 + r]);
        out[2] = g;
    }
}
void launch_fold_ranks(hipStream_t s, const double *t, int nranks, double *out, int do_xn,
                       int do_gn) {
    k_fold_ranks<<<1, 64, 0, s>>>(t, nranks, out, do_xn, do_gn);
}
void launch_param_central(hipStream_t s, const DevProblem &P, const double *x, double *ext_pertB,
                          double *stepB, double delta, double *count, double *c15) {
    if (P.n > 0)
        k_param_central<<<nblk(P.n, 256), 256, 0, s>>>(P, x, ext_pertB, stepB, delta, count,
                                                        c15);
}

template <int NV>
__device__ __forceinline__ void b15_block_sum(double (&v)[NV], double (*red)[1024]) {
    const int tid = threadIdx.x;
#pragma unroll
    for (int k = 0; k < NV; ++k) red[k][tid] = v[k];
    __syncthreads();
    for (int w = 512; w > 0; w >>= 1) {
        if (tid < w) {
#pragma unroll
            for (int k = 0; k < NV; ++k) red[k][tid] += red[k][tid + w];
        }
        __syncthreads();
    }
#pragma unroll
    for (int k = 0; k < NV; ++k) v[k] = red[k][0];
    __syncthreads();
}

__global__ void k_b15_s(const double *fsq, double fn, double *out) {
    if (threadIdx.x == 0) *out = fsq ? *fsq : fn * fn;
}

__global__ void __launch_bounds__(1024) k_b15_combine(
    int n, const double *__restrict__ u, const double *__restrict__ c,
    const double *__restrict__ zu, const double *__restrict__ zc, const double *__restrict__ sp,
    double *xs, double *kinv, double *scalar, int fail_slot, const double *__restrict__ fail_prev) {
    __shared__ double red[4][1024];
    double d[4] = {0., 0., 0., 0.};
    for (int j = threadIdx.x; j < n; j += 1024) {
        d[0] += u[j] * zu[j];
        d[1] += u[j] * zc[j];
        d[2] += c[j] * zu[j];
        d[3] += c[j] * zc[j];
    }
    b15_block_sum<4>(d, red);
    const double s = *sp;
    const double k00 = d[0] - s, k01 = 1. + d[1], k10 = 1. + d[2], k11 = d[3];
    const double det = k00 * k11 - k01 * k10;
    const bool sing = !(fabs(det) > 0.) || !isfinite(det);
    const double i00 = k11 / det, i01 = -k01 / det, i10 = -k10 / det, i11 = k00 / det;
    const double r0 = d[0] + s * d[1], r1 = d[2] + s * d[3];
    const double al = i00 * r0 + i01 * r1, be = i10 * r0 + i11 * r1;
// ... 511 lines not shown
```

mayamatchmovesolver_amd/csrc/mmba_lm.cpp:

```cpp
#include <algorithm>
#include <cfloat>
#include <chrono>
#include <thread>
#include <cmath>
#include <cstdio>
#include <cstring>

#include "mmba_geom.h"
#include "mmba_kernels.h"
#include "mmba_plan.h"

namespace mmba {

constexpr bool kBacksubGroup = true;
constexpr bool kBacksubGroupOnepass = true;

static double wall_now() {
    return std::chrono::duration<double>(std::chrono::steady_clock::now().time_since_epoch())
        .count();
}

hipEvent_t Plan::next_event() {
    if (ev_used == ev_pool.size()) {
        hipEvent_t e = nullptr;
// ... 116 lines not shown
            }
        }
    }
    if (!mirrored)
        MMBA_HIP(hipMemcpyAsync(h_scalar + lo, d_scalar + lo, sizeof(double) * (hi - lo + 1),
                                hipMemcpyDeviceToHost, s));
    if (!spin_wait || (nranks > 1 && comm && comm->bounded())) {
        host_sync();
        return;
    }
    if (!ev_sync) MMBA_HIP(hipEventCreateWithFlags(&ev_sync, hipEventDisableTiming));
    MMBA_HIP(hipEventRecord(ev_sync, s));
    for (;;) {
        const hipError_t e = hipEventQuery(ev_sync);
        if (e == hipSuccess) break;
        if (e != hipErrorNotReady) MMBA_HIP(e);
    }
}

void Plan::stream_wait() {
    if (!ev_sync) MMBA_HIP(hipEventCreateWithFlags(&ev_sync, hipEventDisableTiming));
    MMBA_HIP(hipEventRecord(ev_sync, s));
    wait_event();
}

double Plan::read_scalar(int slot) {
    read_slots(slot, slot);
    return h_scalar[slot];
}

void Plan::allreduce(double *d, size_t count, ReduceOp op) {
    if (comm && nranks > 1) comm->allreduce(d, count, op, s);
}

double Plan::reduce_read(int slot, ReduceOp op) {
    allreduce(d_scalar + slot, 1, op);
    return read_scalar(slot);
}

void Plan::dnorm_enqueue(const double *dv, int slot) {
    launch_sumsq(s, dv, d_diag, n, d_partial, nparts, d_scalar + slot, d_p_own, d_ticket);
    allreduce(d_scalar + slot, 1);
}

double Plan::dnorm(const double *dv) {
    dnorm_enqueue(dv, SL_DNORM);
    return std::sqrt(read_scalar(SL_DNORM));
}

void Plan::records_enqueue(const double *xat, int base_only) {
    launch_records(s, P, d_var_cf, d_ext_pert, d_step, d_recs, nvar, d_brec, base_only);
    recs_full_at = base_only ? nullptr : xat;
}

void Plan::fun_enqueue(const double *dx, double *df, double *eu, double *ed, double *dist,
                       int slot) {
    flush_red();
    launch_param_set(s, P, dx, d_ext, d_ext_pert, d_step, opt.solver_type, opt.delta, fd_eps());
    params_at = dx;
    records_enqueue(dx, 0);
    span_begin(SPAN_RESID);
    launch_rows_eval(s, P, df + 2 * (size_t)M, eu ? eu + 2 * (size_t)M : nullptr, d_partial,
                     (M + 255) / 256);
    launch_residual(s, P, d_recs, df, eu, ed, d_partial, d_scalar + slot,
                    P.nrows > 0 ? nullptr : d_ticket, dist);
    span_end(SPAN_RESID);
    allreduce(d_scalar + slot, 1);
}

double Plan::fun(const double *dx, double *df, double *eu, double *ed, double *dist) {
    const double t0 = wall_now();
    fun_enqueue(dx, df, eu, ed, dist);
    const double r = std::sqrt(read_scalar(SL_FNORM));
    t_func += wall_now() - t0;
    return r;
}

bool Plan::pre_jac_ok() const {
    return pre_jac && nranks == 1 && !central && nrows == 0 && !timing && !k2_split &&
           ne_epilogue_fusable(P) && jac_ne_fusable(P, jac_ncv) && !(cbk && cbk->interrupt) &&
           !(cbk && cbk->progress);
}

void Plan::pre_jac_enqueue(const double *dx, double *eu, double *ed) {
    NeEpi epi;
    epi.on = 1;
    epi.first = 0;
    epi.mode = opt.auto_param_scale == 1 ? 1 : 2;
    epi.fnorm = 0.;
    epi.fnorm_sq = d_scalar + SL_FNORM;
    epi.do_xn = 0;
    epi.do_gn = 1;
    epi.x = dx;
    epi.diag = d_diag;
    epi.acnorm = d_acnorm;
    epi.partial = d_partial;
    epi.rstride = pw;
    epi.cf_base = 0;
    epi.bnd_base = ncf;
    epi.gate = d_gate;
    epi.probe = d_k2probe;
    launch_jac_ne(s, jb_recompute() ? P_nojb() : P, d_recs, d_step, opt.solver_type, d_J, d_jcol,
                  nloc_set ? nullptr : d_nloc, d_stale, eu, ed, d_Acc, d_g, epi);
    nloc_set = true;
    pre_jac_pending = true;
    pre_bnd_pending = false;
    if (P.nbs > 0 && P.JB != nullptr && nG == 0) {
        if (jb_recompute()) {
            epi.jb_recs = d_recs;
            epi.jb_lmder = opt.solver_type == MMBA_SOLVER_CMINPACK_LMDER ? 1 : 0;
        }
        if (fold_ok && nB_solved > 0) {
            epi.Lb = d_Lb;
            epi.tb = d_tb;
            epi.fail = d_fail;
        }
        launch_ne(s, P, d_J, d_jcol, d_nloc, d_f, d_Acc, d_Acg, d_Abb, d_Abg, d_Agg, d_g,
                  d_glob_partial, glob_chunk, epi, true);
        pre_bnd_pending = true;
    }
    pre_sobs_pending = false;
    if (pre_bnd_pending && fold_ok && nB_solved > 0 && !rs_bnd && red_defer_ok() &&
        path_choice(MMBA_PATH_PRE_SCHUR) == 1) {
        const int ncol = ncf + (nB + NE_BND_TPB - 1) / NE_BND_TPB;
        RedSpec rs{};
        rs.flag_slot = -1;
        rs.row[rs.nrows++] = {0, ncol, 1, SL_ZERO};
        rs.row[rs.nrows++] = {2 * pw, ncol, 1, SL_GNORM};
        launch_schur_obs(s, P, d_J, d_Lb, d_W, &rs, d_partial, d_scalar, d_gate);
        pre_sobs_pending = true;
    }
    pre_jac_x = dx;
}

bool Plan::jb_recompute() const {
    return P.JB != nullptr && P.all_bnd_fast && path_choice(MMBA_PATH_JB_RECOMPUTE) == 1;
}

DevProblem Plan::P_nojb() const {
    DevProblem Q = P;
    Q.JB = nullptr;
    return Q;
}

void Plan::jac(const double *dx, const JacLM *lm) {
    flush_red();
    const double t0 = wall_now();
    const double eps_dif = fd_eps();
    const bool lmder = opt.solver_type == MMBA_SOLVER_CMINPACK_LMDER;
    if (params_at != dx) {
        launch_param_set(s, P, dx, d_ext, d_ext_pert, d_step, opt.solver_type, opt.delta, eps_dif);
        recs_full_at = nullptr;
    }
    params_at = dx;
    if (recs_full_at != dx) records_enqueue(dx, 0);
    CentralB CB;
    if (central) {
        MMBA_HIP(hipMemsetAsync(d_scalar + SL_NCENT, 0, sizeof(double), s));
        launch_param_central(s, P, dx, d_ext_pertB, d_stepB, opt.delta, d_scalar + SL_NCENT,
                             b15 ? d_c15 : nullptr);
        launch_records(s, P, d_var_cf, d_ext_pertB, d_stepB, d_recsB, nvar, d_brecB, 0);
        CB.recs = d_recsB;
        CB.brec = d_brecB;
        CB.ext_pert = d_ext_pertB;
        CB.step = d_stepB;
        if (b15) {
            launch_b15_q(s, P, d_c15, d_q15, d_kap15, d_c15r);
            CB.q15 = d_q15;
            CB.kap15 = d_kap15;
        }
    }
    span_begin(SPAN_JAC);
    const bool fuse = lm && ne_epilogue_fusable(P) && nrows == 0 && !b15;
    NeEpi epi;
    if (fuse) {
        epi.on = 1;
        epi.first = lm->first;
        epi.mode = lm->mode;
        epi.fnorm = lm->fnorm;
        epi.fnorm_sq = lm->fnorm_sq;
        epi.do_xn = lm->first;
        epi.do_gn = lm->fnorm_sq || lm->fnorm != 0.;
        epi.x = dx;
        epi.diag = d_diag;
        epi.acnorm = d_acnorm;
        epi.partial = d_partial;
// ... 91 lines not shown
            launch_b15_s(s, lm->fnorm_sq, lm->fnorm, d_b15k + 4);
            launch_b15_unrot(s, P, d_Acc, d_g, d_q15, d_adiag15, d_u15);
        }
        launch_jac_epilogue(s, P, d_Acc, d_Abb, d_Agg, d_acnorm, d_g, d_diag, dx, lm->first,
                            lm->mode, lm->fnorm, lm->fnorm_sq, do_xn, do_gn, d_p_own, d_partial,
                            nparts, pw, b15 ? d_c15 : nullptr, d_b15k + 4, d_g15, d_adiag15,
                            d_u15);
        span_end(SPAN_JAC);
        RedSpec rs{};
        rs.flag_slot = -1;
        rs.row[rs.nrows++] = {0, nparts, 1, SL_ZERO};
        if (do_xn) rs.row[rs.nrows++] = {pw, nparts, 0, SL_XN2};
        if (do_gn) rs.row[rs.nrows++] = {2 * pw, nparts, 1, SL_GNORM};
        if (nranks > 1) {
            double *tail = d_Agg + NGMAX * NGMAX + NGMAX;
            MMBA_HIP(hipMemsetAsync(tail, 0, sizeof(double) * (2 + nranks), s));
            RedSpec rj{};
            rj.flag_slot = -1;
            rj.row[rj.nrows++] = {0, nparts, 1, 0};
            if (do_xn) rj.row[rj.nrows++] = {pw, nparts, 0, 1};
            if (do_gn) rj.row[rj.nrows++] = {2 * pw, nparts, 1, 2 + rank};
            launch_reduce_multi(s, d_partial, rj, tail);
            allreduce(tail, 2 + nranks);
            launch_fold_ranks(s, tail, nranks, d_scalar + SL_ZERO, do_xn, do_gn);
        } else if (red_defer_ok() && !timing) {
            pend_rs = rs;
            pend_red = true;
        } else {
            launch_reduce_multi(s, d_partial, rs, d_scalar);
        }
    }
    t_jac += wall_now() - t0;
}

void Plan::trial_enqueue(double *eu, double *ed, bool with_dnorm, bool fill_dnorm,
                         const LmDec *dec, bool jac_ahead) {
    flush_red();
    const double t0 = wall_now();
    double *pr = d_partial + 3 * (size_t)pw;
    const int tparts = trial_folded     ? trial_fold_parts(P, n_trial_other, trial_rec)
                       : trial_prep_rec ? trial_prep_rec_parts(P, n_prep_other)
                                        : nparts;
    if (!trial_folded && trial_prep_rec) {
        TrialFold T;
        T.x = d_x;
        T.diag = d_diag;
        T.wa1 = d_wa1;
        T.wa2 = d_wa2;
        T.wa3 = d_wa3;
        T.ext = d_ext;
        T.ext_pert = d_ext_pert;
        T.step = d_step;
        T.solver_type = opt.solver_type;
        T.delta = opt.delta;
        T.eps_dif = fd_eps();
        T.other = d_prep_other;
        T.nother = n_prep_other;
        T.partial = pr;
        T.rstride = pw;
        T.own = d_p_own;
        T.rec = 1;
        T.recs = d_recs;
        T.brec = d_brec;
        launch_trial_prep_rec(s, P, d_xs, T);
    } else if (!trial_folded) {
        launch_trial_prep(s, P, d_xs, d_x, d_diag, d_wa1, d_wa2, d_wa3, d_ext, d_ext_pert, d_step,
                          opt.solver_type, opt.delta, fd_eps(), d_p_own, pr, nparts, pw);
    }
    if (b15) launch_b15_rot(s, P, d_q15, d_wa1, d_p15);
    params_at = d_wa2;
    if ((trial_folded && trial_rec) || (!trial_folded && trial_prep_rec))
        recs_full_at = d_wa2;
    else
        records_enqueue(d_wa2, 0);
    span_begin(SPAN_RESID);
    launch_rows_eval(s, P, d_ftrial + 2 * (size_t)M, eu + 2 * (size_t)M, pr + 2 * (size_t)pw,
                     (M + 255) / 256, d_Jrow, d_wa1, pr + 3 * (size_t)pw);
    RedSpec rs{};
    rs.flag_slot = -1;
    rs.row[rs.nrows++] = {3 * pw, tparts, 0, SL_PNORM};
    rs.row[rs.nrows++] = {4 * pw, tparts, 0, SL_XN2T};
    rs.row[rs.nrows++] = {5 * pw, trial_blocks(P), 0, SL_FNORM};
    rs.row[rs.nrows++] = {6 * pw, trial_blocks(P), 0, SL_JP};
    if (fill_dnorm) {
        rs.row[rs.nrows++] = {3 * pw, tparts, 0, SL_DNORM};
        rs.flag_slot = SL_FAIL;
    }
    const bool mirror = host_mirror && nranks == 1;
    RedTail T;
    if (nranks == 1 && tail_reduce) {
        T.on = 1;
        T.spec = rs;
        T.partial = d_partial;
        T.scalar = d_scalar;
        T.flag = fill_dnorm ? d_fail : nullptr;
        T.host = mirror ? h_scalar : nullptr;
        T.host_n = SL_LAST + 1;
        T.ticket = d_mticket;
    }
    launch_residual_jp(s, P, d_recs, d_ftrial, eu, ed, pr + 2 * (size_t)pw, d_J, d_jcol, d_nloc,
                       b15 ? d_p15 : d_wa1, pr + 3 * (size_t)pw, d_dist_t, T);
    span_end(SPAN_RESID);
    LmDec D;
    if (dec) {
        D = *dec;
        D.on = 1;
        D.s_pnorm = SL_PNORM;
        D.s_xn2t = SL_XN2T;
        D.s_fnorm = SL_FNORM;
        D.s_jp = SL_JP;
        D.s_dnorm = SL_DNORM;
        D.s_fail = SL_FAIL;
        D.s_xn2 = SL_XN2;
        D.s_gnorm = SL_GNORM;
        D.s_f0 = SL_F0;
        D.s_out = SL_DGO;
        D.gate = d_gate;
    }
    if (!T.on) {
        const bool sq = mirror && seq_poll;
        if (sq) ++seq_next;
        launch_reduce_multi(s, d_partial, rs, d_scalar, fill_dnorm ? d_fail : nullptr,
                            mirror ? h_scalar : nullptr, SL_LAST + 1, d_mticket,
                            sq ? h_seq : nullptr, seq_next, D);
        seq_pending = sq;
    }
    if (b15)
        launch_b15_jp(s, n, d_xs15r, d_g, d_c15r, d_b15k + 4, d_scalar + SL_JP);
    mirror_pending = mirror;
    pre_hb_enq = dec && pre_hb_on && !b15;
    if (pre_hb_enq)
        MMBA_HIP(hipEventRecord(ev_hb[3], s));
    if (dec && jac_ahead) {
        stage_slots();
        pre_jac_enqueue(d_wa2, eu, ed);
    }
    if (pre_hb_enq) {
        MMBA_HIP(hipStreamWaitEvent(s_hb[0], ev_hb[3], 0));
        launch_handback_host(s_hb[0], Mg, nrows, d_dev_of_ref, d_f, eu, ed, pre_hb_map[0],
                             pre_hb_map[1], pre_hb_map[2], d_scalar + SL_DGO, d_ftrial);
        hb_used[0] = true;
        hb_pending = true;
    }
    allreduce(d_scalar + SL_PNORM, with_dnorm ? 6 : 4);
    t_func += wall_now() - t0;
}

void Plan::solve_damped_enqueue(double lam, int dnorm_slot, bool defer, bool dnorm_by_trial) {
    if (nranks > 1 && path_choice(MMBA_PATH_FAULT_SHARD) == rank + 1)
        throw Invalid{"injected shard fault (MMBA_PATH_FAULT_SHARD)"};
    if (nranks > 1 && path_choice(MMBA_PATH_STALL_SHARD) == rank + 1 && !stall_done) {
        stall_done = true;
        std::this_thread::sleep_for(std::chrono::milliseconds(2 * (long long)comm_timeout_ms()));
    }
    if (!red_defer_ok()) flush_red();
    if (b15 && !b15_inner) {
        b15_inner = true;
        launch_b15_accl(s, P, d_Acc, d_q15, d_diag, lam, d_AccL, d_diagL);
        std::swap(d_Acc, d_AccL);
        std::swap(d_diag, d_diagL);
        solve_damped_enqueue(lam, -1, false, false);
        MMBA_HIP(hipMemcpyAsync(d_z15u, d_xs, sizeof(double) * n, hipMemcpyDeviceToDevice, s));
        MMBA_HIP(hipMemcpyAsync(d_b15k + 5, d_scalar + SL_FAIL, sizeof(double),
                                hipMemcpyDeviceToDevice, s));
        std::swap(d_g, d_c15r);
        solve_damped_enqueue(lam, -1, false, false);
        std::swap(d_g, d_c15r);
        std::swap(d_Acc, d_AccL);
        std::swap(d_diag, d_diagL);
        MMBA_HIP(hipMemcpyAsync(d_z15c, d_xs, sizeof(double) * n, hipMemcpyDeviceToDevice, s));
        b15_inner = false;
        launch_b15_combine(s, n, d_g, d_c15r, d_z15u, d_z15c, d_b15k + 4, d_xs15r, d_b15k,
                           d_scalar, SL_FAIL, d_b15k + 5);
        launch_b15_rot(s, P, d_q15, d_xs15r, d_xs);
        if (dnorm_slot >= 0) launch_b15_dnorm(s, n, d_xs, d_diag, d_scalar + dnorm_slot);
        (void)defer;
        (void)dnorm_by_trial;
        return;
    }
    const double t0 = wall_now();
    trial_folded = false;
    if (band && bs.use_bd && nG == 0 && nranks == 1 && dnorm_slot >= 0) {
        span_begin(SPAN_CHOL);
        bd_direct(s, P, bs.bd, d_Acc, d_g, d_diag, lam, d_xR, d_xs, d_fail, d_scalar, dnorm_slot,
                  SL_FAIL, pend_red ? &pend_rs : nullptr, d_partial);
        pend_red = false;
        span_end(SPAN_CHOL);
        t_linear += wall_now() - t0;
        return;
    }
    if (nB_solved > 0) {
        if (!(lam == 0. && lb0_valid))
            launch_bundle_factor(s, P, d_Abb, d_Abg, d_g, d_diag, lam, d_Lb, d_tb, d_Wg, d_fail);
        const bool ahead = sobs_ahead && lam == 0. && lb0_valid && !rs_bnd;
        sobs_ahead = false;
        lb0_valid = false;
        if (rs_bnd)
            launch_schur_obs_rs(s, PV, M, d_nloc, d_vobs, d_vcoff, d_J, d_Lb, d_W);
        else if (!ahead) {
            launch_schur_obs(s, P, d_J, d_Lb, d_W, pend_red ? &pend_rs : nullptr, d_partial,
                             d_scalar);
            pend_red = false;
        }
    }
    const DevProblem &PS = schur_problem();
    if (nR > 0) {
        const SView V = sview();
        if (nranks > 1) MMBA_HIP(hipMemsetAsync(d_rhs, 0, sizeof(double) * nRpad, s));
        if (band && bs.red) {
            MMBA_HIP(hipMemsetAsync(bs.red, 0, sizeof(double) * (bs.red_count - nRpad), s));
        } else if (band && ((!bs.use_bcr && !bs.use_bd) || rs_bnd)) {
            const int nb = nR - nG;
            MMBA_HIP(hipMemsetAsync(bs.Bd, 0, sizeof(double) * (size_t)nb * (bw + 1), s));
            if (nG > 0) MMBA_HIP(hipMemsetAsync(bs.Ga, 0, sizeof(double) * (size_t)nG * nb, s));
            MMBA_HIP(hipMemsetAsync(bs.Gd, 0, sizeof(double) * NGMAX * NGMAX, s));
        } else if (dense) {
            MMBA_HIP(hipMemsetAsync(d_S, 0, sizeof(double) * (size_t)(nRpad + 1) * dld, s));
        } else if (!band) {
            MMBA_HIP(hipMemsetAsync(d_S, 0, sizeof(double) * (size_t)nslots * TILE * TILE, s));
        }
        const bool fold = fold_init && nB_solved > 0;
        if (!fold) {
            launch_schur_init(s, P, d_Acc, d_Acg, d_Agg, d_g, d_diag, lam, V, nRpad - nR, d_rhs,
                              pend_red ? &pend_rs : nullptr, d_partial, d_scalar);
            pend_red = false;
        }
        flush_red();
        if (nB_solved > 0) {
            if (use_dest) {
                SchurInitFold fi{};
                if (fold) fi = SchurInitFold{1, d_Acc, d_g, d_diag, lam};
                const bool rhs_done =
                    launch_schur_dest(s, PS, d_W, d_dest, d_dest_off, ndest, d_dpairs, V,
                                      pc_uniform, band && bs.use_bcr && !rs_bnd, d_tb, d_rhs, fi,
                                      d_dest_wave, n_dest_wave, d_dest_lane, n_dest_lane);
                if (!rhs_done) launch_schur_rhs(s, PS, d_W, d_tb, d_row_cf, d_rhs);
                launch_schur_glob(s, PS, d_W, d_Wg, d_tb, V, d_rhs);
            } else {
// ... 6 lines not shown
            MMBA_HIP(hipMemcpyAsync(d_rkeep, d_rhs, sizeof(double) * nRpad, hipMemcpyDeviceToDevice,
                                    s));
        }
        span_begin(SPAN_CHOL);
        if (band && bs.use_bd) {
            bd_factor_solve(s, bs.bd, d_fail, d_rhs, d_yR, d_xR, d_xs);
        } else if (band) {
            if (bs.red) allreduce(bs.red, bs.red_count);
            if (bs.use_pcr && !bs.df_off)
                pcr_solve(s, bs.pcr, d_rhs, d_xR, bs.pcr.row_param ? d_xs : nullptr, d_fail);
            else
                band_factor_forward(s, bs, d_fail, d_probe, d_rhs, d_yR);
        } else if (dense) {
            if (nranks > 1) {
                allreduce(d_S, (size_t)ds.ld * (ds.n + 1));
                allreduce(d_rhs, nRpad);
            }
            ds.factor_forward(s, d_rhs, d_yR, d_fail);
        } else {
            for (int k = 0; k < NT; ++k) {
                const int r0 = panel_rows_off[k], nr = panel_rows_off[k + 1] - r0;
                launch_chol_panel(s, d_S, d_slot, NT, k, d_rows + r0, nr, d_Linv, d_fail);
                const int q0 = panel_pairs_off[k], nq = panel_pairs_off[k + 1] - q0;
                launch_chol_update(s, d_S, d_slot, NT, k, d_pairs + q0, nq);
            }
        }
        span_end(SPAN_CHOL);
        if (band && bs.use_bd) {
        } else if (band && bs.use_pcr && !bs.df_off) {
        } else if (band) {
            band_backward(s, bs, d_yR, d_xR);
            if (nranks > 1 && !bs.use_bcr) gather_step_rows();
        } else if (dense) {
            ds.backward(s, d_yR, d_xR);
        } else if (narrow) {
            launch_trsv_fwd_all(s, d_S, d_slot, NT, d_rows_off, d_rows, d_Linv, d_rhs, d_yR);
            launch_trsv_bwd_all(s, d_S, d_slot, NT, d_cols_off, d_cols, d_Linv, d_yR, d_xR);
        } else {
            for (int k = 0; k < NT; ++k) {
                const int r0 = panel_rows_off[k], nr = panel_rows_off[k + 1] - r0;
                launch_trsv_fwd(s, d_S, d_slot, NT, k, d_rows + r0, nr, d_Linv, d_rhs, d_yR);
            }
            for (int k = NT - 1; k >= 0; --k) {
                const int c0 = panel_cols_off[k], nc = panel_cols_off[k + 1] - c0;
                launch_trsv_bwd(s, d_S, d_slot, NT, k, d_cols + c0, nc, d_Linv, d_yR, d_xR);
            }
        }
        const bool pcr_now = band && bs.use_pcr && !bs.df_off;
        if (!(band && ((bs.use_bcr && !pcr_now && bs.bcr.xs) || (pcr_now && bs.pcr.row_param) ||
                       bs.use_bd)))
            launch_scatter_xR(s, P, d_xR, d_xs);
    }
    trial_folded = false;
    if (nB_solved > 0) {
        if (trial_fold_ok) {
            const int gpin = path_choice(MMBA_PATH_BACKSUB_GROUP);
            const int opin = path_choice(MMBA_PATH_BACKSUB_ONEPASS);
            const bool group = !P.rs && !rs_bnd && (gpin < 0 ? kBacksubGroup : gpin == 1);
            const bool onepass = opin < 0 ? (group && kBacksubGroupOnepass) : opin == 1;
            if (!onepass) launch_obs_wtx(s, PS, d_W, d_xR, d_U);
            TrialFold T;
            T.x = d_x;
            T.diag = d_diag;
            T.wa1 = d_wa1;
            T.wa2 = d_wa2;
            T.wa3 = d_wa3;
            T.ext = d_ext;
            T.ext_pert = d_ext_pert;
            T.step = d_step;
            T.solver_type = opt.solver_type;
            T.delta = opt.delta;
            T.eps_dif = fd_eps();
            T.other = d_trial_other;
            T.nother = n_trial_other;
            T.partial = d_partial + 3 * (size_t)pw;
            T.rstride = pw;
            T.own = d_p_own;
            T.rec = trial_rec ? 1 : 0;
            T.recs = d_recs;
            T.brec = d_brec;
            T.group = group ? 1 : 0;
            T.bobs_rp = d_bobs_rp;
            T.brec_fwd = brec_fwd ? 1 : 0;
            launch_backsub_trial(s, PS, onepass ? d_W : nullptr, d_Wg, d_tb, d_Lb, d_xR, d_U, d_xs, T);
            trial_folded = true;
            params_at = nullptr;
            recs_full_at = nullptr;
        } else {
            launch_backsub_bundle(s, PS, d_W, d_Wg, d_tb, d_Lb, d_xR, d_U, d_xs);
        }
    }
    if (dnorm_by_trial) {
        t_linear += wall_now() - t0;
        return;
    }
    if (dnorm_slot < 0) {
        launch_flag_to_scalar(s, d_fail, d_scalar + SL_FAIL);
    } else {
        double *pr = d_partial + 7 * (size_t)pw;
        launch_sumsq(s, d_xs, d_diag, n, pr, nparts, nullptr, d_p_own);
        RedSpec rs{};
        rs.flag_slot = SL_FAIL;
        rs.row[rs.nrows++] = {7 * pw, nparts, 0, dnorm_slot};
        launch_reduce_multi(s, d_partial, rs, d_scalar, d_fail);
    }
    if (dnorm_slot == SL_DNORM) {
        if (!defer) allreduce(d_scalar + SL_DNORM, 2);
    } else {
        if (dnorm_slot >= 0) allreduce(d_scalar + dnorm_slot, 1);
        allreduce(d_scalar + SL_FAIL, 1);
    }
    t_linear += wall_now() - t0;
}

bool Plan::solve_damped(double lam) {
    solve_damped_enqueue(lam);
    return read_scalar(SL_FAIL) == 0.;
}

void Plan::newton_enqueue(double dxnorm) {
    const double t0 = wall_now();
    launch_newton_v(s, n, d_diag, d_xs, dxnorm, d_v);
    if (b15) {
        launch_b15_rot(s, P, d_q15, d_v, d_v15);
        std::swap(d_v, d_v15);
    }
    MMBA_HIP(hipMemsetAsync(d_scalar + SL_NEWT_B, 0, 2 * sizeof(double), s));
    if (nR > 0) launch_gather_R(s, P, d_v, d_wR, nRpad);
    if (nB_solved > 0) {
        launch_newton_bundle(s, schur_problem(), d_W, d_Wg, d_Lb, d_v, d_wR, d_usq, d_nu, d_ngp);
        launch_reduce_sum(s, d_usq, nB, d_scalar + SL_NEWT_B);
    }
    if (nR > 0) {
        if (band && bs.use_pcr && !bs.df_off) {
            pcr_rhs_dot(s, bs.pcr, d_wR, d_ymask, d_fail);
            launch_reduce_sum(s, bs.pcr.part, bs.pcr.nblk, d_scalar + SL_NEWT_R);
        } else if (band && bs.use_bd) {
            bd_forward(s, bs.bd, d_wR, d_yR);
        } else if (band) {
            band_forward(s, bs, d_wR, d_yR);
        } else if (dense) {
            ds.forward(s, d_wR, d_yR);
        } else if (narrow) {
            launch_trsv_fwd_all(s, d_S, d_slot, NT, d_rows_off, d_rows, d_Linv, d_wR, d_yR);
        } else {
            for (int k = 0; k < NT; ++k) {
                const int r0 = panel_rows_off[k], nr = panel_rows_off[k + 1] - r0;
                launch_trsv_fwd(s, d_S, d_slot, NT, k, d_rows + r0, nr, d_Linv, d_wR, d_yR);
            }
        }
        if (band && bs.pcr_int && !bs.df_off)
            launch_sumsq_mix(s, d_yR, d_wR, nR, d_partial, nparts, d_scalar + SL_NEWT_R, d_ymask);
        else if (!(band && bs.use_pcr && !bs.df_off))
            launch_sumsq(s, d_yR, nullptr, nRpad, d_partial, nparts, d_scalar + SL_NEWT_R,
                         d_ymask, d_ticket);
    }
    if (b15) {
        launch_b15_newton(s, n, d_v, d_z15u, d_z15c, d_b15k, d_scalar + SL_NEWT_B);
        std::swap(d_v, d_v15);
    }
    allreduce(d_scalar + SL_NEWT_B, 2);
    t_linear += wall_now() - t0;
}

static void lmpar_first_enqueue(Plan &pl, bool defer = false, bool by_trial = false) {
    pl.solve_damped_enqueue(0.0, Plan::SL_DNORM, defer, by_trial);
// ... 831 lines not shown
```

mayamatchmovesolver_amd/csrc/mmba_plan.h:

```cpp
#pragma once

#include <hip/hip_runtime.h>

#include <algorithm>
#include <cfloat>
#include <cmath>
#include <memory>
#include <string>
#include <vector>

#include "mmba_internal.h"
#include "mmba_kernels.h"

struct mmba_context {
    int device = 0;
    hipStream_t stream = nullptr;
    std::vector<mmba_context *> shards;
    std::vector<mmba::Comm *> comms;
};

namespace mmba {

void set_error(const std::string &msg);
int path_choice(int key);
// ... 237 lines not shown
    template <class T>
    T *upload(const T *src, size_t count) {
        T *d = dalloc<T>(count);
        if (count && src)
            MMBA_HIP(hipMemcpyAsync(d, src, count * sizeof(T), hipMemcpyHostToDevice, s));
        return d;
    }

    void build(const mmba_problem *prob, const mmba_options *o);

    enum Slot {
        SL_PNORM = 0,
        SL_XN2T = 1,
        SL_FNORM = 2,
        SL_JP = 3,
        SL_DNORM = 4,
        SL_FAIL = 5,
        SL_NEWT_B = 6,
        SL_NEWT_R = 7,
        SL_GDIV = 8,
        SL_ZERO = 9,
        SL_XN2 = 10,
        SL_GNORM = 11,
        SL_RMS = 12,
        SL_NCENT = 13,
        SL_F0 = 14,
        SL_DGO = 15,
        SL_DRATIO = 16,
        SL_DDELTA = 17,
        SL_DPAR = 18,
        SL_DINFO = 19,
        SL_LAST = 19,
        SL_FI = 20,
        SL_ESUM = 21,
        SL_ENMIN = 22,
        SL_EMAX = 23,
        SL_IESUM = 24,
        SL_IENMIN = 25,
        SL_IEMAX = 26,
        NSLOT = 28
    };
    void read_slots(int lo, int hi);
    static constexpr bool spin_wait = true;
    hipEvent_t ev_sync = nullptr;
    double read_scalar(int slot = 0);
    void stream_wait();
    void allreduce(double *d, size_t count, ReduceOp op = ReduceOp::Sum);
    double reduce_read(int slot, ReduceOp op = ReduceOp::Sum);
    void fun_enqueue(const double *dx, double *df, double *eu, double *ed,
                     double *dist = nullptr, int slot = SL_FNORM);
    double fun(const double *dx, double *df, double *eu, double *ed, double *dist = nullptr);
    double *d_dist_x = nullptr, *d_dist_t = nullptr;
    std::vector<long long> param_vidx;
    std::vector<double> pmin_h, pmax_h, poff_h, pscale_h;
    void error_stats_device(const double *ed, double *avg, double *mn, double *mx);
    void error_stats_enqueue(const double *ed, int base = SL_ESUM);
    struct JacLM {
        int first, mode;
        double fnorm;
        const double *fnorm_sq = nullptr;
    };
    void jac(const double *dx, const JacLM *lm = nullptr);
    const mmba_callbacks *cbk = nullptr;
    bool poll_interrupt() const {
        return cbk && cbk->interrupt && cbk->interrupt(cbk->user) != 0;
    }
    void jac_partial_stale(const double *dx, int k);
    void trial_enqueue(double *eu, double *ed, bool with_dnorm = false, bool fill_dnorm = false,
                       const LmDec *dec = nullptr, bool jac_ahead = false);
    bool trial_fold_ok = false, trial_folded = false;
    bool trial_rec = false;
    int2 *d_bobs_rp = nullptr;
    bool brec_fwd = false;
    bool trial_prep_rec = false;
    int *d_prep_other = nullptr;
    int n_prep_other = 0;
    int *d_trial_other = nullptr;
    int n_trial_other = 0;
    bool pre_jac = true;
    bool pre_jac_pending = false;
    const double *pre_jac_x = nullptr;
    int *d_gate = nullptr;
    bool pre_jac_ok() const;
    void pre_jac_enqueue(const double *dx, double *eu, double *ed);
    bool slots_staged = false;
    void stage_slots();
    bool pend_red = false;
    RedSpec pend_rs{};
    bool red_defer_ok() const;
    void flush_red();
    void host_sync();
    bool jb_recompute() const;
    DevProblem P_nojb() const;
    bool stall_done = false;
    bool pre_bnd_pending = false;
    bool pre_sobs_pending = false, sobs_ahead = false;
    double *d_cf_part = nullptr;
    unsigned *d_cf_ticket = nullptr;
    void wait_event();
    double *d_eu_s = nullptr, *d_ed_s = nullptr;
    bool spec_ok = true;
    bool outputs_ready = false;
    const double *params_at = nullptr;
    const double *recs_full_at = nullptr;
    bool lb0_valid = false;
    void records_enqueue(const double *xat, int base_only);
    void attrs_reset() {
        MMBA_HIP(hipMemcpyAsync(P.attr_val, d_attr0, attr_bytes, hipMemcpyDeviceToDevice, s));
        params_at = nullptr;
        recs_full_at = nullptr;
    }
    double fd_eps() const { return std::sqrt(std::max(std::fabs(opt.delta), DBL_EPSILON)); }
    int pw = 0;
    void solve_damped_enqueue(double lam, int dnorm_slot = -1, bool defer = false,
                              bool dnorm_by_trial = false);
    bool solve_damped(double lam);
    void newton_enqueue(double dxnorm);
    void dnorm_enqueue(const double *dv, int slot);
    double dnorm(const double *dv);
    int solve(double *x_inout, double *fvec_out, double *eu_out, double *ed_out,
              mmba_result *res, const mmba_callbacks *cb, mmba_trace *trace);
    int solve_once(double *x_inout, double *fvec_out, double *eu_out, double *ed_out,
                   mmba_result *res, const mmba_callbacks *cb, mmba_trace *trace);
    int spec_replays = 0;
    bool batch_ok = false;
    std::string batch_why;
    int batch_nf = 0, batch_nfmax = 0;
    int *d_fr_cf_off = nullptr, *d_fr_par_off = nullptr, *d_fr_par = nullptr,
        *d_fr_last = nullptr, *d_fr_nobs = nullptr;
    double *d_bJ = nullptr, *d_bdist = nullptr, *d_bx = nullptr, *d_bpw = nullptr;
    BatchOut *d_bout = nullptr;
    int *h_bflag = nullptr, *d_bflag = nullptr;
    int solve_frames(double *x_inout, mmba_result *results, const mmba_callbacks *cb);
    int dense_jacobian(const double *x, double *fjac);
    bool dbg_keep_S = false;
    double *d_Skeep = nullptr, *d_rkeep = nullptr;
    int reduced_residual(const double *x, double lam, double *relres);
    bool dbg_jcol_stored = false;
    void assemble_dense_jacobian(double *fjac);
    int damped_step(const double *x, double lam, double *step_out, double *g_out,
                    double *diag_out, double *fjac_out);
    int reproject(const double *x, double *point_out, double *marker_out);
    int measure(const double *x, double *fvec_out, double *eu_out, double *ed_out,
                double *stats);
    void download_params(const double *dx, double *x_out);
    void download_ref_order(const double *d_f2, const double *d_eu2, const double *d_ed1,
                            double *f_out, double *eu_out, double *ed_out, bool sync = true);
    hipStream_t s_hb[3] = {nullptr, nullptr, nullptr};
    hipEvent_t ev_hb[4] = {nullptr, nullptr, nullptr, nullptr};
    bool hb_pending = false;
    bool hb_used[3] = {false, false, false};
    void handback_wait();
    void handback_streams();
    bool map_outputs(double *f_out, double *eu_out, double *ed_out, double *hmap[3]);
    bool pre_hb_on = false, pre_hb_enq = false;
    long long pre_handbacks = 0;
    long long ne_split_launches = 0;
    double *pre_hb_map[3] = {nullptr, nullptr, nullptr};
};

}

namespace mmba {
struct ShardGroup;
void destroy_group(ShardGroup *g);
struct GroupDeleter {
    void operator()(ShardGroup *g) const { destroy_group(g); }
};
}

namespace mmba {
int group_plan_create(mmba_context *ctx, const mmba_problem *prob, const mmba_options *opt,
                      mmba_plan **out);
int group_plan_solve(mmba_plan *plan, double *x_inout, double *fvec_out, double *err_user_out,
                     double *err_dist_out, mmba_result *res, const mmba_callbacks *cb,
                     mmba_trace *trace);
int group_plan_measure(mmba_plan *plan, const double *x, double *fvec_out, double *err_user_out,
                       double *err_dist_out, double *avg_min_max_out);
int group_plan_reproject(mmba_plan *plan, const double *x, double *point_xy_out,
                         double *marker_xy_out);
int group_plan_jacobian(mmba_plan *plan, const double *x, double *fjac);
int group_plan_outputs(mmba_plan *plan, double *fvec_out, double *err_user_out,
                       double *err_dist_out);
int group_plan_set_attr_values(mmba_plan *plan, const double *attr_values);
int group_plan_solve_per_frame(mmba_plan *plan, double *x_inout, mmba_result *results,
                               const mmba_callbacks *cb);
int group_plan_kernel_stats(mmba_plan *plan, int enable_timing, mmba_kernel_stats *out);
}

struct mmba_plan {
    mmba::Plan impl;
    std::unique_ptr<mmba::ShardGroup, mmba::GroupDeleter> group;
};
```

Baseline: 2.104 billion residuals/s.

## Fold trial reduction and LM decision into the speculative Jacobian/NE kernel

```diff
diff --git a/include/mmba.h b/include/mmba.h
--- a/include/mmba.h
+++ b/include/mmba.h
@@ -284,6 +284,7 @@
     double chol_flops_alg;
     int32_t pre_handbacks;
     int32_t ne_split_launches;
+    int32_t trial_red_folds;
 } mmba_kernel_stats;
 int mmba_plan_kernel_stats(mmba_plan *plan, int enable_timing,
                            mmba_kernel_stats *out);
@@ -312,7 +313,8 @@
 #define MMBA_PATH_PRE_HANDBACK 22
 #define MMBA_PATH_PRE_SCHUR 23
 #define MMBA_PATH_BACKSUB_GROUP 24
-#define MMBA_PATH_NUM 25
+#define MMBA_PATH_TRIAL_RED_FOLD 25
+#define MMBA_PATH_NUM 26
 int mmba_debug_set_path(int key, int value);
 
 int mmba_debug_band_solve(mmba_context *ctx, int nb, int w, int nG, int P, const double *S,
diff --git a/mayamatchmovesolver_amd/abi.py b/mayamatchmovesolver_amd/abi.py
--- a/mayamatchmovesolver_amd/abi.py
+++ b/mayamatchmovesolver_amd/abi.py
@@ -43,7 +43,8 @@
 PATH_PRE_HANDBACK = 22
 PATH_PRE_SCHUR = 23
 PATH_BACKSUB_GROUP = 24
-PATH_NUM = 25
+PATH_TRIAL_RED_FOLD = 25
+PATH_NUM = 26
 
 FILM_FIT_FILL = 0
 FILM_FIT_HORIZONTAL = 1
@@ -228,6 +229,7 @@
         ("chol_flops_alg", C.c_double),
         ("pre_handbacks", C.c_int32),
         ("ne_split_launches", C.c_int32),
+        ("trial_red_folds", C.c_int32),
     ]
 
     def as_dict(self):
diff --git a/mayamatchmovesolver_amd/csrc/mmba_api.cpp b/mayamatchmovesolver_amd/csrc/mmba_api.cpp
--- a/mayamatchmovesolver_amd/csrc/mmba_api.cpp
+++ b/mayamatchmovesolver_amd/csrc/mmba_api.cpp
@@ -12,9 +12,10 @@
 static thread_local std::string g_last_error;
 void set_error(const std::string &msg) { g_last_error = msg; }
 
-static_assert(MMBA_PATH_NUM == 25, "one initialiser per path key");
+static_assert(MMBA_PATH_NUM == 26, "one initialiser per path key");
 static std::atomic<int> g_path[MMBA_PATH_NUM] = {-1, -1, -1, -1, -1, -1, -1, -1, -1, -1, -1, -1, -1,
-                                                 -1, -1, -1, -1, -1, -1, -1, -1, -1, -1, -1, -1};
+                                                 -1, -1, -1, -1, -1, -1, -1, -1, -1, -1, -1, -1,
+                                                 -1};
 int path_choice(int key) {
     return (key > 0 && key < MMBA_PATH_NUM) ? g_path[key].load() : -1;
 }
@@ -404,6 +405,7 @@
         out->spec_replays = p.spec_replays;
         out->pre_handbacks = (int32_t)p.pre_handbacks;
         out->ne_split_launches = (int32_t)p.ne_split_launches;
+        out->trial_red_folds = (int32_t)p.trial_red_folds;
         {
             const BandSolver &b = p.bs;
             out->band_solver = !p.band ? 0
diff --git a/mayamatchmovesolver_amd/csrc/mmba_kernels.h b/mayamatchmovesolver_amd/csrc/mmba_kernels.h
--- a/mayamatchmovesolver_amd/csrc/mmba_kernels.h
+++ b/mayamatchmovesolver_amd/csrc/mmba_kernels.h
@@ -129,10 +129,22 @@
     const int *gate = nullptr;
     long long *probe = nullptr;
 };
+struct TrialRed {
+    int on = 0;
+    RedSpec spec{};
+    LmDec dec{};
+    const double *partial = nullptr;
+    double *scalar = nullptr;
+    double *host = nullptr;
+    int host_n = 0;
+    unsigned *host_seq = nullptr;
+    unsigned seq = 0;
+};
 bool jac_ne_fusable(const DevProblem &P, int ncv);
 void launch_jac_ne(hipStream_t s, const DevProblem &P, const double *recs, const double *step,
                    int solver_type, double *J, int *jcol, int *nloc, const int *stale_param,
-                   double *eu, double *ed, double *Acc, double *g, const NeEpi &E);
+                   double *eu, double *ed, double *Acc, double *g, const NeEpi &E,
+                   const TrialRed &R = TrialRed());
 bool ne_epilogue_fusable(const DevProblem &P);
 bool launch_ne(hipStream_t s, const DevProblem &P, const double *J, const int *jcol,
                const int *nloc, const double *f, double *Acc, double *Acg, double *Abb,
@@ -203,6 +215,8 @@
     int group = 0;
     const int2 *bobs_rp = nullptr;
     int brec_fwd = 0;
+    int *flag = nullptr;
+    double *flag_out = nullptr;
 };
 bool trial_records_ok(const DevProblem &P);
 int trial_fold_parts(const DevProblem &P, int nother, bool rec = false);
diff --git a/mayamatchmovesolver_amd/csrc/mmba_kernels.hip b/mayamatchmovesolver_amd/csrc/mmba_kernels.hip
--- a/mayamatchmovesolver_amd/csrc/mmba_kernels.hip
+++ b/mayamatchmovesolver_amd/csrc/mmba_kernels.hip
@@ -116,26 +116,34 @@
     }
 }
 
-__device__ __forceinline__ double reduce_row_w64(const double *partial, const RedRow &rw) {
+constexpr int RED_JB = 6;
+struct RowQ {
+    double q[4][RED_JB];
+};
+__device__ __forceinline__ void row_issue(const double *partial, const RedRow &rw, RowQ &Q) {
+    const int t = threadIdx.x & 63;
+    if (rw.n <= 256 * RED_JB) {
+#pragma unroll
+        for (int k = 0; k < 4; ++k)
+#pragma unroll
+            for (int j = 0; j < RED_JB; ++j) {
+                const int i = t + 64 * k + 256 * j;
+                Q.q[k][j] = i < rw.n ? partial[rw.off + i] : 0.;
+            }
+    }
+}
+__device__ __forceinline__ double row_finish(const double *partial, const RedRow &rw,
+                                             const RowQ &Q) {
     const bool mx = rw.is_max != 0;
     const int t = threadIdx.x & 63;
     double s[4];
-    constexpr int JB = 6;
-    if (rw.n <= 256 * JB) {
-        double q[4][JB];
-#pragma unroll
-        for (int k = 0; k < 4; ++k)
-#pragma unroll
-            for (int j = 0; j < JB; ++j) {
-                const int i = t + 64 * k + 256 * j;
-                q[k][j] = i < rw.n ? partial[rw.off + i] : 0.;
-            }
+    if (rw.n <= 256 * RED_JB) {
 #pragma unroll
         for (int k = 0; k < 4; ++k) {
             double v = 0.;
 #pragma unroll
-            for (int j = 0; j < JB; ++j)
-                if (t + 64 * k + 256 * j < rw.n) v = mx ? fmax(v, q[k][j]) : v + q[k][j];
+            for (int j = 0; j < RED_JB; ++j)
+                if (t + 64 * k + 256 * j < rw.n) v = mx ? fmax(v, Q.q[k][j]) : v + Q.q[k][j];
             s[k] = v;
         }
     } else {
@@ -158,6 +166,96 @@
         if (t < w) r = mx ? fmax(r, o) : r + o;
     }
     return r;
+}
+__device__ __forceinline__ double reduce_row_w64(const double *partial, const RedRow &rw) {
+    RowQ Q;
+    row_issue(partial, rw, Q);
+    return row_finish(partial, rw, Q);
+}
+
+struct LmIn {
+    double f0, xn2, gnorm, fail, dnorm, pnorm, fnorm, jp, xn2t;
+};
+struct LmOut {
+    int go, info;
+    double ratio, delta, par;
+};
+__device__ __forceinline__ LmOut lm_decide_vals(const LmDec &d, const LmIn &v) {
+    const double p1 = .1, p5 = .5, p25 = .25, p75 = .75, p0001 = 1e-4;
+    const double epsmch = DBL_EPSILON;
+    double fnorm = d.f0 ? sqrt(v.f0) : d.fnorm;
+    double delta = d.delta, xnorm = d.xnorm, par = d.par, gnorm = d.gnorm;
+    int info = 0, go = 0;
+    double ratio = 0.;
+    bool taken = true;
+    if (d.spec) {
+        if (d.first) {
+            xnorm = sqrt(v.xn2);
+            delta = d.factor * xnorm;
+            if (delta == 0.) delta = d.factor;
+        }
+        gnorm = fnorm != 0. ? v.gnorm : 0.;
+        if (gnorm <= d.gtol) {
+            info = 4;
+            taken = false;
+        } else {
+            const double fl = v.fail;
+            const bool ok0 = fl == 0.;
+            const double dxnorm = ok0 ? sqrt(v.dnorm) : HUGE_VAL;
+            const double fp = dxnorm - delta;
+            taken = fl < 2. && fp <= p1 * delta;
+            par = 0.;
+        }
+    }
+    if (taken) {
+        const double pnorm = sqrt(v.pnorm);
+        if (d.first) delta = fmin(delta, pnorm);
+        const double fnorm1 = sqrt(v.fnorm);
+        double actred = -1.;
+        if (p1 * fnorm1 < fnorm) {
+            const double d1 = fnorm1 / fnorm;
+            actred = 1. - d1 * d1;
+        }
+        const double temp1 = sqrt(v.jp) / fnorm;
+        const double temp2 = (sqrt(par) * pnorm) / fnorm;
+        const double prered = temp1 * temp1 + temp2 * temp2 / p5;
+        const double dirder = -(temp1 * temp1 + temp2 * temp2);
+        if (prered != 0.) ratio = actred / prered;
+        if (ratio <= p25) {
+            double temp;
+            if (actred >= 0.)
+                temp = p5;
+            else
+                temp = p5 * dirder / (dirder + p5 * actred);
+            if (p1 * fnorm1 >= fnorm || temp < p1) temp = p1;
+            delta = temp * fmin(delta, pnorm / p1);
+            par /= temp;
+        } else if (par == 0. || ratio >= p75) {
+            delta = pnorm / p5;
+            par = p5 * par;
+        }
+        const bool accept = ratio >= p0001;
+        if (accept) xnorm = sqrt(v.xn2t);
+        if (fabs(actred) <= d.ftol && prered <= d.ftol && p5 * ratio <= 1.) info = 1;
+        if (delta <= d.xtol * xnorm) info = 2;
+        if (fabs(actred) <= d.ftol && prered <= d.ftol && p5 * ratio <= 1. && info == 2) info = 3;
+        if (info == 0) {
+            if (d.nfev >= d.maxfev) info = 5;
+            if (fabs(actred) <= epsmch && prered <= epsmch && p5 * ratio <= 1.) info = 6;
+            if (delta <= epsmch * xnorm) info = 7;
+            if (gnorm <= epsmch) info = 8;
+        }
+        go = (accept && info == 0) ? 1 : 0;
+    }
+    return LmOut{go, taken ? info : -100 - info, ratio, delta, par};
+}
+__device__ __forceinline__ void lm_publish(const LmDec &d, const LmOut &o, double *scalar) {
+    scalar[d.s_out] = o.go;
+    scalar[d.s_out + 1] = o.ratio;
+    scalar[d.s_out + 2] = o.delta;
+    scalar[d.s_out + 3] = o.par;
+    scalar[d.s_out + 4] = o.info;
+    __hip_atomic_store(d.gate, o.go, __ATOMIC_RELAXED, __HIP_MEMORY_SCOPE_AGENT);
 }
 
 constexpr int RED_ROWS = 8;
@@ -1024,13 +1122,13 @@
 };
 template <int PC>
 __device__ __forceinline__ EpiPre epi_preload(const DevProblem &P, const NeEpi &E, int cf,
-                                              int lane) {
+                                              int lane, bool own = false, double fsq_own = 0.) {
     EpiPre q{-1, 0., 0., 0.};
     if (!E.on || lane >= PC) return q;
     q.p = P.cf_var_param[P.cf_var_off[cf] + 1 + lane];
     q.dg = E.diag[q.p];
     if (E.do_xn) q.xv = E.x[q.p];
-    if (E.do_gn) q.fn = E.fnorm_sq ? sqrt(*E.fnorm_sq) : E.fnorm;
+    if (E.do_gn) q.fn = own ? sqrt(fsq_own) : E.fnorm_sq ? sqrt(*E.fnorm_sq) : E.fnorm;
     return q;
 }
 __device__ __forceinline__ void epi_param_pre(const NeEpi &E, const EpiPre &q, double d, double gp,
@@ -1281,46 +1379,152 @@
 }
 
 
+
+__device__ __forceinline__ void jac_ne_publish(const TrialRed &R, const LmIn &v, const LmOut &o) {
+    if (threadIdx.x == 0) {
+        const double val[5] = {v.pnorm, v.xn2t, v.fnorm, v.jp, v.dnorm};
+#pragma unroll
+        for (int r = 0; r < 5; ++r)
+            if (r < R.spec.nrows) R.scalar[R.spec.row[r].slot] = val[r];
+        lm_publish(R.dec, o, R.scalar);
+    }
+    if (!R.host) return;
+    if (threadIdx.x < 64) {
+        __builtin_amdgcn_fence(__ATOMIC_SEQ_CST, "workgroup");
+        for (int i = threadIdx.x; i < R.host_n; i += 64)
+            R.host[i] = __hip_atomic_load(&R.scalar[i], __ATOMIC_RELAXED, __HIP_MEMORY_SCOPE_AGENT);
+        if (R.host_seq) {
+            __threadfence_system();
+            if (threadIdx.x == 0)
+                __hip_atomic_store(R.host_seq, R.seq, __ATOMIC_RELEASE, __HIP_MEMORY_SCOPE_SYSTEM);
+        }
+    }
+}
+
+struct TrialRows {
+    RowQ Q0, Q1;
+    int r0, nred;
+    bool dn_dup;
+};
+template <int NW>
+__device__ __forceinline__ void trial_rows_issue(const TrialRed &R, LmIn &tin, TrialRows &T) {
+    const LmDec &d = R.dec;
+    const int nr = R.spec.nrows;
+    T.dn_dup = nr == 5 && R.spec.row[4].off == R.spec.row[0].off &&
+               R.spec.row[4].n == R.spec.row[0].n &&
+               R.spec.row[4].is_max == R.spec.row[0].is_max;
+    T.nred = T.dn_dup ? 4 : nr;
+    T.r0 = __builtin_amdgcn_readfirstlane((int)threadIdx.x >> 6);
+    if (T.r0 < T.nred) row_issue(R.partial, R.spec.row[T.r0], T.Q0);
+    if constexpr (NW == 2)
+        if (T.r0 + NW < T.nred) row_issue(R.partial, R.spec.row[T.r0 + NW], T.Q1);
+    tin.f0 = R.scalar[d.s_f0];
+    tin.xn2 = R.scalar[d.s_xn2];
+    tin.gnorm = R.scalar[d.s_gnorm];
+    tin.fail = R.scalar[d.s_fail];
+    if (nr < 5) tin.dnorm = R.scalar[d.s_dnorm];
+}
+template <int NW>
+__device__ __forceinline__ void trial_rows_finish(const TrialRed &R, double *sTr,
+                                                  const TrialRows &T) {
+    const bool l0 = (threadIdx.x & 63) == 0;
+    if (T.r0 < T.nred) {
+        const double v = row_finish(R.partial, R.spec.row[T.r0], T.Q0);
+        if (l0) sTr[T.r0] = v;
+    }
+    if constexpr (NW == 2)
+        if (T.r0 + NW < T.nred) {
+            const double v = row_finish(R.partial, R.spec.row[T.r0 + NW], T.Q1);
+            if (l0) sTr[T.r0 + NW] = v;
+        }
+    for (int r = T.r0 + (NW == 2 ? 2 : 1) * NW; r < T.nred; r += NW) {
+        const double v = reduce_row_w64(R.partial, R.spec.row[r]);
+        if (l0) sTr[r] = v;
+    }
+}
+__device__ __forceinline__ LmOut trial_decide(const TrialRed &R, const double *sTr, LmIn &tin,
+                                              bool dn_dup) {
+    tin.pnorm = sTr[0];
+    tin.xn2t = sTr[1];
+    tin.fnorm = sTr[2];
+    tin.jp = sTr[3];
+    if (R.spec.nrows == 5) tin.dnorm = dn_dup ? sTr[0] : sTr[4];
+    return lm_decide_vals(R.dec, tin);
+}
+
 template <int PC, int NW, bool GEN>
 __global__ void __launch_bounds__(64 * NW) k_jac_ne_u(
     DevProblem P, const double *__restrict__ recs, const double *__restrict__ step,
     int solver_type, double *__restrict__ J, int *__restrict__ jcol, int *__restrict__ nloc,
     const int *__restrict__ stale_param, double *__restrict__ eu, double *__restrict__ ed,
-    double *Acc, double *g, NeEpi E) {
+    double *Acc, double *g, NeEpi E, TrialRed R) {
     constexpr int NCC = PC * (PC + 1) / 2, NE = NCC + PC;
     __shared__ double wsum[NW][NE];
     __shared__ double sRec[(PC + 1) * CAMREC];
     __shared__ int sPv[PC];
     __shared__ double sSt[PC];
     __shared__ int sHdr[3];
-    if (E.gate && __hip_atomic_load(E.gate, __ATOMIC_RELAXED, __HIP_MEMORY_SCOPE_AGENT) == 0)
+    __shared__ double sTr[5];
+    if (!R.on && E.gate &&
+        __hip_atomic_load(E.gate, __ATOMIC_RELAXED, __HIP_MEMORY_SCOPE_AGENT) == 0)
         return;
-    const int cf = xcd_remap(blockIdx.x, gridDim.x);
+    const int tid = threadIdx.x, lane = tid & 63, wv = tid >> 6;
+    LmIn tin{};
+    TrialRows TR;
+    TR.dn_dup = false;
+    const int pad = R.on ? 8 : 0;
+    const int ncf = (int)gridDim.x - pad;
+    if ((int)blockIdx.x < pad) {
+        if (blockIdx.x != 0) return;
+        trial_rows_issue<NW>(R, tin, TR);
+        trial_rows_finish<NW>(R, sTr, TR);
+        __syncthreads();
+        const LmOut out = trial_decide(R, sTr, tin, TR.dn_dup);
+        jac_ne_publish(R, tin, out);
+        return;
+    }
+    const int cf = xcd_remap((int)blockIdx.x - pad, ncf);
     long long *pr = (E.probe && threadIdx.x == 0) ? E.probe + 5 * (size_t)cf : nullptr;
-    if (pr) pr[0] = (long long)wall_clock64();
+    const long long t_in = pr ? (long long)wall_clock64() : 0;
     const int o0 = P.cf_obs_off[cf], o1 = P.cf_obs_off[cf + 1];
-    const int tid = threadIdx.x, lane = tid & 63, wv = tid >> 6;
     const bool lmder = solver_type == MMBA_SOLVER_CMINPACK_LMDER;
     const bool solved = P.cf_pc[cf] == PC && own_cf(P, cf);
     {
+        constexpr int KT = ((PC + 1) * CAMREC + 64 * NW - 1) / (64 * NW);
         const int voff = P.cf_var_off[cf];
         const int nv = min(P.cf_var_off[cf + 1] - voff - 1, PC);
-        for (int t = tid; t < (nv + 1) * CAMREC; t += 64 * NW)
-            sRec[t] = recs[(size_t)voff * CAMREC + t];
+        double rv[KT];
+#pragma unroll
+        for (int k = 0; k < KT; ++k) {
+            const int t = tid + 64 * NW * k;
+            rv[k] = t < (nv + 1) * CAMREC ? recs[(size_t)voff * CAMREC + t] : 0.;
+        }
+        const int p = (tid < PC && tid < nv) ? P.cf_var_param[voff + 1 + tid] : -1;
+        const int fr = P.cf_frame[cf];
+        if (R.on) trial_rows_issue<NW>(R, tin, TR);
+        const double stv = p >= 0 ? step[p] : 1.;
+#pragma unroll
+        for (int k = 0; k < KT; ++k) {
+            const int t = tid + 64 * NW * k;
+            if (t < (nv + 1) * CAMREC) sRec[t] = rv[k];
+        }
         if (tid < PC) {
-            const int p = tid < nv ? P.cf_var_param[voff + 1 + tid] : -1;
             sPv[tid] = p;
-            sSt[tid] = tid < nv ? step[p] : 1.;
+            sSt[tid] = stv;
         }
         if (tid == 0) {
-            const int fr = P.cf_frame[cf];
             sHdr[0] = nv;
             sHdr[1] = fr;
             sHdr[2] = stale_param[fr];
         }
     }
+    if (R.on) trial_rows_finish<NW>(R, sTr, TR);
     __syncthreads();
-    if (pr) pr[1] = (long long)wall_clock64();
+    if (R.on && trial_decide(R, sTr, tin, TR.dn_dup).go == 0) return;
+    if (pr) {
+        pr[0] = t_in;
+        pr[1] = (long long)wall_clock64();
+    }
     JacCf<PC> C;
     C.rcf = sRec;
 #pragma unroll
@@ -1393,7 +1597,7 @@
                 gp += wsum[w][NCC + ln];
             }
         }
-        epi_params_wave<PC>(P, E, cf, ln, d, gp, epi_preload<PC>(P, E, cf, ln));
+        epi_params_wave<PC>(P, E, cf, ln, d, gp, epi_preload<PC>(P, E, cf, ln, R.on != 0, sTr[2]));
     }
     if (pr) {
         pr[3] = (long long)wall_clock64();
@@ -1881,78 +2085,10 @@
 }
 
 __device__ void lm_decide(const LmDec &d, double *scalar) {
-    const double p1 = .1, p5 = .5, p25 = .25, p75 = .75, p0001 = 1e-4;
-    const double epsmch = DBL_EPSILON;
-    double fnorm = d.f0 ? sqrt(scalar[d.s_f0]) : d.fnorm;
-    double delta = d.delta, xnorm = d.xnorm, par = d.par, gnorm = d.gnorm;
-    int info = 0, go = 0;
-    double ratio = 0.;
-    bool taken = true;
-    if (d.spec) {
-        if (d.first) {
-            xnorm = sqrt(scalar[d.s_xn2]);
-            delta = d.factor * xnorm;
-            if (delta == 0.) delta = d.factor;
-        }
-        gnorm = fnorm != 0. ? scalar[d.s_gnorm] : 0.;
-        if (gnorm <= d.gtol) {
-            info = 4;
-            taken = false;
-        } else {
-            const double fl = scalar[d.s_fail];
-            const bool ok0 = fl == 0.;
-            const double dxnorm = ok0 ? sqrt(scalar[d.s_dnorm]) : HUGE_VAL;
-            const double fp = dxnorm - delta;
-            taken = fl < 2. && fp <= p1 * delta;
-            par = 0.;
-        }
-    }
-    if (taken) {
-        const double pnorm = sqrt(scalar[d.s_pnorm]);
-        if (d.first) delta = fmin(delta, pnorm);
-        const double fnorm1 = sqrt(scalar[d.s_fnorm]);
-        double actred = -1.;
-        if (p1 * fnorm1 < fnorm) {
-            const double d1 = fnorm1 / fnorm;
-            actred = 1. - d1 * d1;
-        }
-        const double temp1 = sqrt(scalar[d.s_jp]) / fnorm;
-        const double temp2 = (sqrt(par) * pnorm) / fnorm;
-        const double prered = temp1 * temp1 + temp2 * temp2 / p5;
-        const double dirder = -(temp1 * temp1 + temp2 * temp2);
-        if (prered != 0.) ratio = actred / prered;
-        if (ratio <= p25) {
-            double temp;
-            if (actred >= 0.)
-                temp = p5;
-            else
-                temp = p5 * dirder / (dirder + p5 * actred);
-            if (p1 * fnorm1 >= fnorm || temp < p1) temp = p1;
-            delta = temp * fmin(delta, pnorm / p1);
-            par /= temp;
-        } else if (par == 0. || ratio >= p75) {
-            delta = pnorm / p5;
-            par = p5 * par;
-        }
-        const bool accept = ratio >= p0001;
-        if (accept) xnorm = sqrt(scalar[d.s_xn2t]);
-        if (fabs(actred) <= d.ftol && prered <= d.ftol && p5 * ratio <= 1.) info = 1;
-        if (delta <= d.xtol * xnorm) info = 2;
-        if (fabs(actred) <= d.ftol && prered <= d.ftol && p5 * ratio <= 1. && info == 2) info = 3;
-        if (info == 0) {
-            if (d.nfev >= d.maxfev) info = 5;
-            if (fabs(actred) <= epsmch && prered <= epsmch && p5 * ratio <= 1.) info = 6;
-            if (delta <= epsmch * xnorm) info = 7;
-            if (gnorm <= epsmch) info = 8;
-        }
-        go = (accept && info == 0) ? 1 : 0;
-    }
-    scalar[d.s_out] = go;
-    scalar[d.s_out + 1] = ratio;
-    scalar[d.s_out + 2] = delta;
-    scalar[d.s_out + 3] = par;
-    scalar[d.s_out + 4] = taken ? info : -100 - info;
-    __hip_atomic_store(d.gate, go, __ATOMIC_RELAXED, __HIP_MEMORY_SCOPE_AGENT);
+    const LmIn v{scalar[d.s_f0],    scalar[d.s_xn2],   scalar[d.s_gnorm],
+                 scalar[d.s_fail],  scalar[d.s_dnorm], scalar[d.s_pnorm],
+                 scalar[d.s_fnorm], scalar[d.s_jp],    scalar[d.s_xn2t]};
+    lm_publish(d, lm_decide_vals(d, v), scalar);
 }
 
 __global__ void __launch_bounds__(256) k_reduce_multi(const double *__restrict__ partial,
@@ -2733,6 +2869,11 @@
     }
 }
 
+__device__ __forceinline__ void backsub_flag(const TrialFold &T) {
+    *T.flag_out = (double)*T.flag;
+    *T.flag = 0;
+}
+
 __global__ void __launch_bounds__(64) k_backsub_trial(DevProblem P, const double *__restrict__ U,
                                                       const double *__restrict__ W,
                                                       const double *__restrict__ Wg,
@@ -2742,6 +2883,7 @@
                                                       int nbb, TrialFold T) {
     __shared__ double red[256];
     double pn = 0., xn = 0.;
+    if (T.flag && blockIdx.x == 0 && threadIdx.x == 0) backsub_flag(T);
     if ((int)blockIdx.x < nbb) {
         const int b = xcd_remap(blockIdx.x, nbb) * blockDim.x + threadIdx.x;
         const int pb = b < P.nB ? P.bnd_pb[b] : 0;
@@ -2874,6 +3016,7 @@
                                                          int nbb, int nob, TrialFold T) {
     __shared__ double red[128];
     const int tid = threadIdx.x;
+    if (T.flag && blockIdx.x == 0 && tid == 0) backsub_flag(T);
     const int pad = (nob + 7) & ~7;
     if ((int)blockIdx.x >= nob && (int)blockIdx.x < pad) return;
     const int bb = (int)blockIdx.x - pad, ob = (int)blockIdx.x;
@@ -3744,13 +3887,15 @@
 }
 void launch_jac_ne(hipStream_t s, const DevProblem &P, const double *recs, const double *step,
                    int solver_type, double *J, int *jcol, int *nloc, const int *stale_param,
-                   double *eu, double *ed, double *Acc, double *g, const NeEpi &E) {
+                   double *eu, double *ed, double *Acc, double *g, const NeEpi &E,
+                   const TrialRed &R) {
     if (P.ncf == 0) return;
+    const int grid = P.ncf + (R.on ? 8 : 0);
     const long long per = (P.M + P.ncf - 1) / P.ncf;
     int nw = per > 1024 ? 8 : (per > 256 ? 4 : 2);
 #define MMBA_JN(PC, NW, GEN)                                                                  \
-    k_jac_ne_u<PC, NW, GEN><<<P.ncf, 64 * NW, 0, s>>>(P, recs, step, solver_type, J, jcol, nloc, \
-                                                        stale_param, eu, ed, Acc, g, E)
+    k_jac_ne_u<PC, NW, GEN><<<grid, 64 * NW, 0, s>>>(P, recs, step, solver_type, J, jcol, nloc, \
+                                                       stale_param, eu, ed, Acc, g, E, R)
 #define MMBA_JN_NW(PC, GEN)                                         \
     do {                                                            \
         if (nw == 8) MMBA_JN(PC, 8, GEN);                           \
diff --git a/mayamatchmovesolver_amd/csrc/mmba_lm.cpp b/mayamatchmovesolver_amd/csrc/mmba_lm.cpp
--- a/mayamatchmovesolver_amd/csrc/mmba_lm.cpp
+++ b/mayamatchmovesolver_amd/csrc/mmba_lm.cpp
@@ -222,7 +222,12 @@
            !(cbk && cbk->progress);
 }
 
-void Plan::pre_jac_enqueue(const double *dx, double *eu, double *ed) {
+bool Plan::trial_red_fold() const {
+    const int pin = path_choice(MMBA_PATH_TRIAL_RED_FOLD);
+    return pin < 0 ? kTrialRedFold : pin != 0;
+}
+
+void Plan::pre_jac_enqueue(const double *dx, double *eu, double *ed, const TrialRed &red) {
     NeEpi epi;
     epi.on = 1;
     epi.first = 0;
@@ -241,7 +246,7 @@
     epi.gate = d_gate;
     epi.probe = d_k2probe;
     launch_jac_ne(s, jb_recompute() ? P_nojb() : P, d_recs, d_step, opt.solver_type, d_J, d_jcol,
-                  nloc_set ? nullptr : d_nloc, d_stale, eu, ed, d_Acc, d_g, epi);
+                  nloc_set ? nullptr : d_nloc, d_stale, eu, ed, d_Acc, d_g, epi, red);
     nloc_set = true;
     pre_jac_pending = true;
     pre_bnd_pending = false;
@@ -499,9 +504,10 @@
     rs.row[rs.nrows++] = {4 * pw, tparts, 0, SL_XN2T};
     rs.row[rs.nrows++] = {5 * pw, trial_blocks(P), 0, SL_FNORM};
     rs.row[rs.nrows++] = {6 * pw, trial_blocks(P), 0, SL_JP};
+    int *const flag = fill_dnorm && !fail_early ? d_fail : nullptr;
     if (fill_dnorm) {
         rs.row[rs.nrows++] = {3 * pw, tparts, 0, SL_DNORM};
-        rs.flag_slot = SL_FAIL;
+        if (flag) rs.flag_slot = SL_FAIL;
     }
     const bool mirror = host_mirror && nranks == 1;
     RedTail T;
@@ -510,7 +516,7 @@
         T.spec = rs;
         T.partial = d_partial;
         T.scalar = d_scalar;
-        T.flag = fill_dnorm ? d_fail : nullptr;
+        T.flag = flag;
         T.host = mirror ? h_scalar : nullptr;
         T.host_n = SL_LAST + 1;
         T.ticket = d_mticket;
@@ -534,23 +540,37 @@
         D.s_out = SL_DGO;
         D.gate = d_gate;
     }
-    if (!T.on) {
+    const bool hb_enq = dec && pre_hb_on && !b15;
+    TrialRed R;
+    if (dec && jac_ahead && nranks == 1 && !b15 && mirror && seq_poll && !hb_enq && !timing &&
+        !T.on && !flag && trial_red_fold()) {
+        R.on = 1;
+        R.spec = rs;
+        R.dec = D;
+        R.partial = d_partial;
+        R.scalar = d_scalar;
+        R.host = h_scalar;
+        R.host_n = SL_LAST + 1;
+        R.host_seq = h_seq;
+        R.seq = ++seq_next;
+        seq_pending = true;
+        ++trial_red_folds;
+    } else if (!T.on) {
         const bool sq = mirror && seq_poll;
         if (sq) ++seq_next;
-        launch_reduce_multi(s, d_partial, rs, d_scalar, fill_dnorm ? d_fail : nullptr,
-                            mirror ? h_scalar : nullptr, SL_LAST + 1, d_mticket,
-                            sq ? h_seq : nullptr, seq_next, D);
+        launch_reduce_multi(s, d_partial, rs, d_scalar, flag, mirror ? h_scalar : nullptr,
+                            SL_LAST + 1, d_mticket, sq ? h_seq : nullptr, seq_next, D);
         seq_pending = sq;
     }
     if (b15)
         launch_b15_jp(s, n, d_xs15r, d_g, d_c15r, d_b15k + 4, d_scalar + SL_JP);
     mirror_pending = mirror;
-    pre_hb_enq = dec && pre_hb_on && !b15;
+    pre_hb_enq = hb_enq;
     if (pre_hb_enq)
         MMBA_HIP(hipEventRecord(ev_hb[3], s));
     if (dec && jac_ahead) {
         stage_slots();
-        pre_jac_enqueue(d_wa2, eu, ed);
+        pre_jac_enqueue(d_wa2, eu, ed, R);
     }
     if (pre_hb_enq) {
         MMBA_HIP(hipStreamWaitEvent(s_hb[0], ev_hb[3], 0));
@@ -571,6 +591,7 @@
         std::this_thread::sleep_for(std::chrono::milliseconds(2 * (long long)comm_timeout_ms()));
     }
     if (!red_defer_ok()) flush_red();
+    fail_early = false;
     if (b15 && !b15_inner) {
         b15_inner = true;
         launch_b15_accl(s, P, d_Acc, d_q15, d_diag, lam, d_AccL, d_diagL);
@@ -743,6 +764,11 @@
             T.group = group ? 1 : 0;
             T.bobs_rp = d_bobs_rp;
             T.brec_fwd = brec_fwd ? 1 : 0;
+            if (dnorm_by_trial && nranks == 1 && !b15 && trial_red_fold()) {
+                T.flag = d_fail;
+                T.flag_out = d_scalar + SL_FAIL;
+                fail_early = true;
+            }
             launch_backsub_trial(s, PS, onepass ? d_W : nullptr, d_Wg, d_tb, d_Lb, d_xR, d_U, d_xs, T);
             trial_folded = true;
             params_at = nullptr;
diff --git a/mayamatchmovesolver_amd/csrc/mmba_plan.h b/mayamatchmovesolver_amd/csrc/mmba_plan.h
--- a/mayamatchmovesolver_amd/csrc/mmba_plan.h
+++ b/mayamatchmovesolver_amd/csrc/mmba_plan.h
@@ -343,7 +343,11 @@
     const double *pre_jac_x = nullptr;
     int *d_gate = nullptr;
     bool pre_jac_ok() const;
-    void pre_jac_enqueue(const double *dx, double *eu, double *ed);
+    void pre_jac_enqueue(const double *dx, double *eu, double *ed,
+                         const TrialRed &red = TrialRed());
+    static constexpr bool kTrialRedFold = true;
+    bool trial_red_fold() const;
+    bool fail_early = false;
     bool slots_staged = false;
     void stage_slots();
     bool pend_red = false;
@@ -417,6 +421,7 @@
     bool pre_hb_on = false, pre_hb_enq = false;
     long long pre_handbacks = 0;
     long long ne_split_launches = 0;
+    long long trial_red_folds = 0;
     double *pre_hb_map[3] = {nullptr, nullptr, nullptr};
 };
 
```

Result: faster. 2.133 billion residuals/s (median of 6 runs) (+1.4%).
